# vrenkens/tfkaldi

Measured on AMD Instinct MI355X. Metric: acoustic frames/sec (train step), higher is better.
Workload: dtype f32 emulated (3xbf16 planes, 6 products, f32 accumulate)

## Files before the change

### tfkaldi_amd/csrc/gemm_bf16.hip

```cpp
#include "gemm_bf16.h"
#include "x3_layout.h"

#include <math.h>
#include <stdlib.h>
#include <string.h>

#include <type_traits>

namespace tfk {
namespace {

typedef __bf16 bf16x8 __attribute__((ext_vector_type(8)));
typedef __bf16 bf16x4 __attribute__((ext_vector_type(4)));
typedef float f32x16 __attribute__((ext_vector_type(16)));
typedef uint32_t u32x4 __attribute__((ext_vector_type(4)));
typedef int i32x4 __attribute__((ext_vector_type(4)));

constexpr int BK = 64;
constexpr int kOOB = (int)0x80000000;
constexpr int NUM_XCD = 8;

__device__ __forceinline__ void tile_of_block(int tiles_m, int tiles_n, int group_rows, int bid, int& tm, int& tn) {
  const int nwg = tiles_m * tiles_n;
  const int xcd = bid % NUM_XCD, loc = bid / NUM_XCD;
  const int q = nwg / NUM_XCD, r = nwg % NUM_XCD;
  const int seq = (xcd < r ? xcd * (q + 1) : r * (q + 1) + (xcd - r) * q) + loc;
  const int per_group = group_rows * tiles_n;
  const int grp = seq / per_group;
  const int first_m = grp * group_rows;
  const int gsize = min(group_rows, tiles_m - first_m);
  const int within = seq - grp * per_group;
  tm = first_m + within % gsize;
  tn = within / gsize;
}

__device__ __forceinline__ uint16_t f2bf(float x) { return __builtin_bit_cast(uint16_t, (__bf16)x); }

template <int EPI, int WAVES_M, int WAVES_N, int FM, int FN>
__device__ __forceinline__ void epilogue(const GemmArgsB& p, f32x16 (&acc)[FM][FN], int tiles_m, int tm, int m0, int n0,
                                         int wm, int wn, int i, int h, float* red) {
  constexpr int BM = WAVES_M * FM * 32, BN = WAVES_N * FN * 32;
  auto row_of = [&](int a, int r) { return m0 + (wm * FM + a) * 32 + 4 * h + (r & 3) + 8 * (r >> 2); };
#pragma unroll
  for (int b = 0; b < FN; ++b) {
    const int cidx = (wn * FN + b) * 32 + i;
    const int col = n0 + cidx;
    const bool col_ok = col < p.N;
    const int colc = col_ok ? col : p.N - 1;
    if constexpr ((EPI & EPI_BIAS) != 0) {
      const float bv = p.bias[colc];
#pragma unroll
      for (int a = 0; a < FM; ++a)
#pragma unroll
        for (int r = 0; r < 16; ++r) acc[a][b][r] += bv;
    }
    if constexpr ((EPI & EPI_EVAL_ACT) != 0) {
      const bool bn = p.act_mean != nullptr;
      const float mu = bn ? p.act_mean[colc] : 0.f;
      const float rs = bn ? rsqrtf(p.act_rstd[colc] + p.bn_eps) : 1.f;
      const float be = bn ? p.act_beta[colc] : 0.f;
#pragma unroll
      for (int a = 0; a < FM; ++a)
#pragma unroll
        for (int r = 0; r < 16; ++r) {
          float u = acc[a][b][r];
          if (bn) u = (u - mu) * rs + be;
          switch (p.act_nonlin) {
            case 0: u = fmaxf(u, 0.f); break;
            case 1: u = 1.f / (1.f + expf(-u)); break;
            case 2: u = tanhf(u); break;
            default: break;
          }
          acc[a][b][r] = u;
        }
    }
    if constexpr ((EPI & EPI_COLSTATS) != 0) {
      const int vlim = p.row_vend ? min(p.M, p.row_vend[m0 >> 6]) : p.M;
      const int n_tile = max(1, min(BM, vlim - m0));
      float cmean = 0.f;
#pragma unroll
      for (int pass = 0; pass < 2; ++pass) {
        float s = 0.f;
#pragma unroll
        for (int a = 0; a < FM; ++a)
#pragma unroll
          for (int r = 0; r < 16; ++r) {
            const float v = acc[a][b][r];
            if (row_of(a, r) < vlim) s += pass == 0 ? v : (v - cmean) * (v - cmean);
          }
        s += __shfl_xor(s, 32);
        if (h == 0) red[wm * BN + cidx] = s;
        __syncthreads();
        float t = 0.f;
#pragma unroll
        for (int w = 0; w < WAVES_M; ++w) t += red[w * BN + cidx];
        if (pass == 0) {
          cmean = t / (float)n_tile;
        } else if (wm == 0 && h == 0 && col_ok) {
          p.stats[((size_t)0 * tiles_m + tm) * p.ldc + col] = cmean;
          p.stats[((size_t)1 * tiles_m + tm) * p.ldc + col] = t;
        }
        __syncthreads();
      }
    }
    if constexpr ((EPI & EPI_DACT) != 0) {
      const float mu = p.act_mean[colc], rsd = p.act_rstd[colc];
      const float dscale = p.act_scale > 0.f ? p.act_scale : 1.f;
      const bool from_a = p.act_nonlin == 0 && p.act_beta != nullptr;
      const float be = from_a ? p.act_beta[colc] : 0.f;
      const float keep = p.act_keep > 0.f ? p.act_keep : 1.f;
      float s1 = 0.f, s2 = 0.f;
#pragma unroll
      for (int a = 0; a < FM; ++a) {
        float av[16], zv[16];
#pragma unroll
        for (int r = 0; r < 16; ++r) {
          const int row = min(row_of(a, r), p.M - 1);
          av[r] = p.act_a[(size_t)row * p.ldc + colc];
        }
        if (!from_a) {
#pragma unroll
          for (int r = 0; r < 16; ++r) {
            const int row = min(row_of(a, r), p.M - 1);
            zv[r] = p.act_z[(size_t)row * p.ldc + colc];
          }
        }
#pragma unroll
        for (int r = 0; r < 16; ++r) {
          float d1;
          switch (p.act_nonlin) {
            case 0: d1 = av[r] > 0.f ? dscale : 0.f; break;
            case 1: d1 = av[r] * (1.f - av[r]); break;
            case 2: d1 = 1.f - av[r] * av[r]; break;
            default: d1 = 1.f;
          }
          const float du = acc[a][b][r] * d1;
          acc[a][b][r] = du;
          if (row_of(a, r) < p.M) {
            s1 += du;
            s2 += du * (from_a ? av[r] * keep - be : (zv[r] - mu) * rsd);
          }
        }
      }
      s1 += __shfl_xor(s1, 32);
      s2 += __shfl_xor(s2, 32);
      if (h == 0) {
        red[(0 * WAVES_M + wm) * BN + cidx] = s1;
        red[(1 * WAVES_M + wm) * BN + cidx] = s2;
      }
      __syncthreads();
      if (wm == 0 && h == 0 && col_ok) {
        float t1 = 0.f, t2 = 0.f;
#pragma unroll
        for (int w = 0; w < WAVES_M; ++w) {
          t1 += red[(0 * WAVES_M + w) * BN + cidx];
          t2 += red[(1 * WAVES_M + w) * BN + cidx];
        }
        p.stats[((size_t)0 * p.stats_stride + tm) * p.ldc + col] = t1;
        p.stats[((size_t)1 * p.stats_stride + tm) * p.ldc + col] = t2;
      }
      __syncthreads();
    }
#pragma unroll
    for (int a = 0; a < FM; ++a) {
      float old[16];
      if constexpr ((EPI & EPI_ACCUM) != 0) {
#pragma unroll
        for (int r = 0; r < 16; ++r) old[r] = p.C[(size_t)min(row_of(a, r), p.M - 1) * p.ldc + colc];
      }
#pragma unroll
      for (int r = 0; r < 16; ++r) {
        const int row = row_of(a, r);
        float v = acc[a][b][r];
        if (EPI & EPI_ACCUM) v += old[r];
        if (col_ok && row < p.M) {
          p.C[(size_t)row * p.ldc + col] = v;
          if constexpr ((EPI & EPI_EVAL_ACT) != 0) {
            if (p.C_twin) {
              if (p.ct_x3) {
                const size_t at = x3::at((size_t)row, col, p.ldct);
                uint16_t q0, q1, q2;
                x3::split3(v, q0, q1, q2);
                p.C_twin[at] = (bf16_t)q0;
                p.C_twin[at + 64] = (bf16_t)q1;
                p.C_twin[at + 128] = (bf16_t)q2;
              } else {
                p.C_twin[(size_t)row * p.ldct + col] = f2bf(v);
              }
            }
          }
        }
      }
    }
  }
}


template <int EXT>
__device__ __forceinline__ int ks_swz(int r) {
  return EXT == 64 ? (((r >> 1) & 1) << 2) : ((r & 3) << 2);
}

template <bool KC, int EXT, int NTH, int BKT = 64>
struct DmaOperand {
  static_assert(BKT == 64 || BKT == 32, "ring slot of 64 or 32 k");
  static constexpr int NP = EXT * BKT / 8 / NTH;
  static_assert((EXT * BKT / 8) % NTH == 0 && NP >= 1, "pieces per thread");
  i32x4 rsrc;
  int voff[NP];
  int kidx[NP];
  int kstride;
  int k_lim;

  __device__ __forceinline__ void init(const bf16_t* base, int ld, int rows, int ext0, int ext_lim, int k_lim_,
                                       int tid, long extra_bytes = 0) {
    const unsigned long long a = (unsigned long long)base;
    rsrc[0] = (int)(unsigned)a;
    rsrc[1] = (int)((unsigned)(a >> 32) & 0xffffu);
    rsrc[2] = (int)(rows * ld * 2 + extra_bytes);
    rsrc[3] = 0x00020000;
    k_lim = k_lim_;
    kstride = KC ? 2 : ld * 2;
#pragma unroll
    for (int j = 0; j < NP; ++j) {
      const int idx = tid + j * NTH;
      if (KC) {
        constexpr int CPR = BKT / 8;
        const int r = idx / CPR;
        const int sw = BKT == 64 ? ((r >> 1) & 7) : ((r >> 2) & 3);
        const int k = ((idx % CPR) ^ sw) << 3;
        const int e = ext0 + r;
        voff[j] = e < ext_lim ? (e * ld + k) * 2 : kOOB;
        kidx[j] = k;
      } else {
        constexpr int CH = EXT / 8;
        const int r = idx / CH;
        const int c = (idx % CH) ^ ks_swz<EXT>(r);
        const int e = ext0 + (c << 3);
        voff[j] = e < ext_lim ? (r * ld + e) * 2 : kOOB;
        kidx[j] = r;
      }
    }
  }
  __device__ __forceinline__ void issue(int j, unsigned image, int k0, int wave, int plane_bytes = 0) const {
    const int off = (k0 + kidx[j] < k_lim) ? voff[j] : kOOB;
    const unsigned dst = image + (unsigned)(wave * 64 + j * NTH) * 16u;
    const int soff = k0 * kstride + plane_bytes;
    asm volatile("s_mov_b32 m0, %0\n\ts_nop 0\n\tbuffer_load_dwordx4 %1, %2, %3 offen lds"
                 :
                 : "s"(dst), "v"(off), "s"(rsrc), "s"(soff)
                 : "memory");
  }
};

template <bool KC, int EXT, int NF, int BKT = 64>
struct Frag {
  int off[KC ? 4 : NF];
  __device__ __forceinline__ void init(int lane, int frag0) {
    if constexpr (KC) {
      const int i = lane & 31, kb = lane >> 5, sw = BKT == 64 ? ((i >> 1) & 7) : ((i >> 2) & 3);
#pragma unroll
      for (int ks = 0; ks < BKT / 16; ++ks) off[ks] = (frag0 * 32 + i) * (BKT * 2) + ((((2 * ks + kb) ^ sw)) << 4);
    } else {
      constexpr int ROWB = EXT * 2;
      const int kb = lane >> 5, half = (lane >> 4) & 1, j = (lane >> 2) & 3, q = lane & 3;
      const int jj = EXT == 64 ? (j >> 1) : j;
#pragma unroll
      for (int f = 0; f < NF; ++f)
        off[f] = (8 * kb + j) * ROWB + ((4 * ((frag0 + f) ^ jj) + 2 * half + (q >> 1)) << 4) + ((q & 1) << 3);
    }
  }
  __device__ __forceinline__ bf16x8 read(const char* img, int f, int ks) const {
    if constexpr (KC) {
      return *reinterpret_cast<const bf16x8*>(img + off[ks] + f * 32 * (BKT * 2));
    } else {
      constexpr int ROWB = EXT * 2;
      typedef __attribute__((address_space(3))) bf16x4 lds_bf16x4;
      const char* q = img + off[f] + ks * 16 * ROWB;
      const bf16x4 lo = __builtin_amdgcn_ds_read_tr16_b64_v4bf16((lds_bf16x4*)q);
      const bf16x4 hi = __builtin_amdgcn_ds_read_tr16_b64_v4bf16((lds_bf16x4*)(q + 4 * ROWB));
      return __builtin_shufflevector(lo, hi, 0, 1, 2, 3, 4, 5, 6, 7);
    }
  }
};

template <bool KC, int EXT, int NTH>
struct DmaOperand3 {
  static constexpr int NP = EXT * 12 / NTH;
  static_assert((EXT * 12) % NTH == 0 && NP >= 1, "pieces per thread");
  i32x4 rsrc;
  int voff[NP];
  int kidx[NP];
  int kstride;
  int k_lim;

  __device__ __forceinline__ void init(const bf16_t* base, int ld, int rows, int ext0, int ext_lim, int k_lim_, int tid) {
    const unsigned long long a = (unsigned long long)base;
    rsrc[0] = (int)(unsigned)a;
    rsrc[1] = (int)((unsigned)(a >> 32) & 0xffffu);
    rsrc[2] = (int)(x3::elems((size_t)rows, ld) * 2);
    rsrc[3] = 0x00020000;
    k_lim = k_lim_;
    kstride = KC ? 12 : ld * 6;
#pragma unroll
    for (int j = 0; j < NP; ++j) {
      const int n = tid + j * NTH;
      if (KC) {
        int r, q, c;
        x3::kc_decode(n, r, q, c);
        const int e = ext0 + r;
        voff[j] = e < ext_lim ? (int)(x3::at((size_t)e, c * 8, ld) + q * 64) * 2 : kOOB;
        kidx[j] = c * 8;
      } else {
        int r, b, q, e8;
        x3::ks_decode<EXT>(n, r, b, q, e8);
        const int e = ext0 + b * 32 + e8 * 8;
        voff[j] = e < ext_lim ? (int)(x3::at((size_t)r, e, ld) + q * 64) * 2 : kOOB;
        kidx[j] = r;
      }
    }
  }
  template <bool GUARD>
  __device__ __forceinline__ void issue(int j, unsigned image, int k0, int wave) const {
    const int off = (!GUARD || k0 + kidx[j] < k_lim) ? voff[j] : kOOB;
    const unsigned dst = image + (unsigned)(wave * 64 + j * NTH) * 16u;
    const int soff = k0 * kstride;
    asm volatile("s_mov_b32 m0, %0\n\ts_nop 0\n\tbuffer_load_dwordx4 %1, %2, %3 offen lds"
                 :
                 : "s"(dst), "v"(off), "s"(rsrc), "s"(soff)
                 : "memory");
  }
};

template <bool KC, int EXT, int NF>
struct Frag3 {
  int off[2];
  __device__ __forceinline__ void init(int lane, int frag0) {
#pragma unroll
    for (int v = 0; v < 2; ++v) off[v] = KC ? x3::kc_lane_off(lane, frag0, v) : x3::ks_lane_off<EXT>(lane, frag0, v);
  }
  __device__ __forceinline__ Frag3 at(int bytes) const {
    Frag3 r;
    r.off[0] = off[0] + bytes;
    r.off[1] = off[1] + bytes;
    return r;
  }
  __device__ __forceinline__ bf16x8 read(const char* img, int f, int ks, int pl) const {
    if constexpr (KC) {
      return *reinterpret_cast<const bf16x8*>(img + off[ks] + x3::kc_imm(f, pl));
    } else {
      typedef __attribute__((address_space(3))) bf16x4 lds_bf16x4;
      const int X = 3 * f + pl;
      const char* q = img + off[X & 1];
      const bf16x4 lo = __builtin_amdgcn_ds_read_tr16_b64_v4bf16((lds_bf16x4*)(q + x3::ks_imm<EXT>(X, ks, 0)));
      const bf16x4 hi = __builtin_amdgcn_ds_read_tr16_b64_v4bf16((lds_bf16x4*)(q + x3::ks_imm<EXT>(X, ks, 1)));
      return __builtin_shufflevector(lo, hi, 0, 1, 2, 3, 4, 5, 6, 7);
    }
  }
};

template <bool KC, int EXT, int NF16>
struct Frag3M {
  int off[KC ? 1 : 4];
  __device__ __forceinline__ void init(int lane, int frag0) {
    if constexpr (KC) {
      off[0] = x3::kc16_lane_off(lane, frag0);
    } else {
#pragma unroll
      for (int v = 0; v < 4; ++v) off[v] = x3::ks16_lane_off<EXT>(lane, frag0, v & 1, v >> 1);
    }
  }
  __device__ __forceinline__ Frag3M at(int bytes) const {
    Frag3M r;
#pragma unroll
    for (int v = 0; v < (KC ? 1 : 4); ++v) r.off[v] = off[v] + bytes;
    return r;
  }
  __device__ __forceinline__ bf16x8 read(const char* img, int f, int pl) const {
    if constexpr (KC) {
      return *reinterpret_cast<const bf16x8*>(img + off[0] + x3::kc16_imm(f, pl));
    } else {
      typedef __attribute__((address_space(3))) bf16x4 lds_bf16x4;
      const int X = 3 * (f >> 1) + pl;
      const char* q = img + off[(X & 1) + 2 * (f & 1)];
      const bf16x4 lo = __builtin_amdgcn_ds_read_tr16_b64_v4bf16((lds_bf16x4*)(q + x3::ks16_imm<EXT>(X, 0)));
      const bf16x4 hi = __builtin_amdgcn_ds_read_tr16_b64_v4bf16((lds_bf16x4*)(q + x3::ks16_imm<EXT>(X, 1)));
      return __builtin_shufflevector(lo, hi, 0, 1, 2, 3, 4, 5, 6, 7);
    }
  }
};

#ifndef TFKB_ABL
#define TFKB_ABL 0
#endif

#define TFKB_WAIT_BARRIER(n) \
  asm volatile("s_waitcnt vmcnt(%0)\n\ts_waitcnt lgkmcnt(0)\n\ts_barrier" : : "n"(n) : "memory")

constexpr int kSplitFlagWords = 4096;
constexpr int kSplitXccWord = 2048;
template <bool A_KC, bool B_KC, int EPI, int WAVES_M, int WAVES_N, int FM, int FN, int NS, int BKT = 64, int SCHED = 0,
          int NPL = 1, int KSPLIT = 1, int LOADERS = 0>
__device__ __forceinline__ void dma_tile(const GemmArgsB& p, int tiles_m, int tiles_n, int group_rows, int bid, char* smem) {
  static_assert(LOADERS == 0 || (NPL == 3 && LOADERS == WAVES_M * WAVES_N), "loader waves: one per multiplying wave, x3 only");
  constexpr int NTH = WAVES_M * WAVES_N * 64;
  constexpr int BM = WAVES_M * FM * 32, BN = WAVES_N * FN * 32;
  typedef typename std::conditional<NPL == 3, DmaOperand3<A_KC, BM, NTH>, DmaOperand<A_KC, BM, NTH, BKT>>::type OA;
  typedef typename std::conditional<NPL == 3, DmaOperand3<B_KC, BN, NTH>, DmaOperand<B_KC, BN, NTH, BKT>>::type OB;
  constexpr int A_BYTES = BM * BKT * 2, B_BYTES = BN * BKT * 2, STAGE = NPL * (A_BYTES + B_BYTES);
  constexpr int NPA = OA::NP, NPB = OB::NP, NP = OA::NP + OB::NP;
  constexpr int KSPT = BKT / 16;
  static_assert(KSPT == 4 || KSPT == 2, "ring slot of 64 or 32 k");
  static_assert(NS >= 3 && (NS - 2) * NP + (NPL == 3 ? NP / 2 : 0) <= 63, "ring depth / vmcnt range");
  static_assert(FM * FN >= 2 || NPL == 3, "two independent accumulator chains per wave");
  static_assert(NPL == 1 || (NPL == 3 && SCHED == 0), "planes");
  static_assert(KSPLIT == 1 || (KSPLIT == 2 && NPL == 3), "split-K: the fp32-emulating contraction only");

  const int tid = threadIdx.x;
  const int lane = tid & 63;
  const int i = lane & 31, h = lane >> 5;
  const int wave = __builtin_amdgcn_readfirstlane(tid >> 6);
  const int wm = wave / WAVES_N, wn = wave % WAVES_N;
  int tm, tn;
  const int khalf = KSPLIT == 2 ? (bid / NUM_XCD) & 1 : 0;
  const int tile_bid = KSPLIT == 2 ? (bid / NUM_XCD >> 1) * NUM_XCD + bid % NUM_XCD : bid;
  tile_of_block(tiles_m, tiles_n, group_rows, tile_bid, tm, tn);
  const int m0 = tm * BM, n0 = tn * BN;
  unsigned my_xcc = 0;
  if constexpr (KSPLIT == 2) {
    if (p.splitk_local) {
      asm volatile("s_getreg_b32 %0, hwreg(HW_REG_XCC_ID, 0, 4)" : "=s"(my_xcc));
      if (tid == 0)
        __hip_atomic_store(reinterpret_cast<unsigned*>(p.splitk_ws) + kSplitXccWord + 2 * (tm * tiles_n + tn) + khalf, my_xcc + 1,
                           __ATOMIC_RELAXED, __HIP_MEMORY_SCOPE_AGENT);
    }
  }

  const int K8 = (p.K + 7) & ~7;
  const int nk_all = (p.K + BKT - 1) / BKT;
  const int h0 = KSPLIT == 2 ? max(1, (nk_all + 1) / 2 - p.splitk_skew) : nk_all;
  const int kbase = khalf ? h0 : 0;
  const int nk = KSPLIT == 2 ? (khalf ? nk_all - h0 : h0) : nk_all;
  const int k_end = (kbase + nk) * BKT;
  const unsigned lds0 = __builtin_amdgcn_readfirstlane((unsigned)(unsigned long long)smem);
  OA la;
  OB lb;
  const int a_klim = min(A_KC ? K8 : p.K, k_end), b_klim = min(B_KC ? K8 : p.K, k_end);
  const int nk_full = min(a_klim, b_klim) / BKT - kbase;
  if constexpr (LOADERS > 0) {
    if (wave >= WAVES_M * WAVES_N) {
      const int lwave = wave - WAVES_M * WAVES_N;
      la.init(p.A, p.lda, A_KC ? p.M : p.K, m0, A_KC ? p.M : ((p.M + 7) & ~7), a_klim, tid - NTH);
      lb.init(p.B, p.ldb, B_KC ? p.N : p.K, n0, B_KC ? p.N : ((p.N + 7) & ~7), b_klim, tid - NTH);
      auto tile = [&](auto guard, int slot, int kt) {
        if (TFKB_ABL & 2) return;
#pragma unroll
        for (int j = 0; j < NPA; ++j)
          la.template issue<decltype(guard)::value>(j, lds0 + (unsigned)(slot * STAGE), (kt + kbase) * BKT, lwave);
#pragma unroll
        for (int j = 0; j < NPB; ++j)
          lb.template issue<decltype(guard)::value>(j, lds0 + (unsigned)(slot * STAGE + NPL * A_BYTES), (kt + kbase) * BKT, lwave);
      };
#pragma unroll
      for (int t = 0; t < NS - 1; ++t) tile(std::true_type(), t, t);
      TFKB_WAIT_BARRIER((NS - 2) * NP);
      int ws = NS - 1;
      const int n_fast = max(0, min(nk, nk_full - (NS - 1)));
#pragma unroll 1
      for (int kt = 0; kt < nk; ++kt) {
        if (kt < n_fast) tile(std::false_type(), ws, kt + NS - 1);
        else tile(std::true_type(), ws, kt + NS - 1);
        TFKB_WAIT_BARRIER((NS - 2) * NP);
        ws = ws + 1 == NS ? 0 : ws + 1;
      }
      TFKB_WAIT_BARRIER(0);
      return;
    }
  } else {
    la.init(p.A, p.lda, A_KC ? p.M : p.K, m0, A_KC ? p.M : ((p.M + 7) & ~7), a_klim, tid);
    lb.init(p.B, p.ldb, B_KC ? p.N : p.K, n0, B_KC ? p.N : ((p.N + 7) & ~7), b_klim, tid);
  }
  typename std::conditional<NPL == 3, Frag3<A_KC, BM, FM>, Frag<A_KC, BM, FM, BKT>>::type qa;
  typename std::conditional<NPL == 3, Frag3<B_KC, BN, FN>, Frag<B_KC, BN, FN, BKT>>::type qb;
  qa.init(lane, wm * FM);
  qb.init(lane, wn * FN);

  f32x16 acc[FM][FN];
  f32x16 acc2[NPL == 3 ? FM : 1][NPL == 3 ? FN : 1];
#pragma unroll
  for (int a = 0; a < FM; ++a)
#pragma unroll
    for (int b = 0; b < FN; ++b)
#pragma unroll
      for (int r = 0; r < 16; ++r) acc[a][b][r] = 0.f;
  if constexpr (NPL == 3) {
#pragma unroll
    for (int a = 0; a < FM; ++a)
#pragma unroll
      for (int b = 0; b < FN; ++b)
#pragma unroll
        for (int r = 0; r < 16; ++r) acc2[a][b][r] = 0.f;
  }

  auto piece_g = [&](auto guard, int j, int slot, int kt) {
    if (TFKB_ABL & 2) return;
    if constexpr (LOADERS > 0) {
      return;
    } else if constexpr (NPL == 3) {
      if (j < NPA)
        la.template issue<decltype(guard)::value>(j, lds0 + (unsigned)(slot * STAGE), (kt + kbase) * BKT, wave);
      else
        lb.template issue<decltype(guard)::value>(j - NPA, lds0 + (unsigned)(slot * STAGE + NPL * A_BYTES), (kt + kbase) * BKT, wave);
    } else {
      if (j < NPA)
        la.issue(j, lds0 + (unsigned)(slot * STAGE), (kt + kbase) * BKT, wave);
      else
        lb.issue(j - NPA, lds0 + (unsigned)(slot * STAGE + A_BYTES), (kt + kbase) * BKT, wave);
    }
  };
  auto piece = [&](int j, int slot, int kt) { piece_g(std::true_type(), j, slot, kt); };
#pragma unroll
  for (int t = 0; t < NS - 1; ++t)
#pragma unroll
    for (int j = 0; j < NP; ++j) piece(j, t, t);
  constexpr int NPH = NPL == 3 ? NP / 2 : 0;
#pragma unroll
  for (int j = 0; j < NPH; ++j) piece(j, NS - 1, NS - 1);
  TFKB_WAIT_BARRIER((NS - 2) * NP + NPH);

  bf16x8 fa[2][NPL][FM], fb[2][NPL][FN];
  auto read_frags = [&](int buf, const char* st, int ks) {
    if (TFKB_ABL & 4) return;
#pragma unroll
    for (int pl = 0; pl < NPL; ++pl) {
      if constexpr (NPL == 3) {
#pragma unroll
        for (int a = 0; a < FM; ++a) fa[buf][pl][a] = qa.read(st, a, ks, pl);
#pragma unroll
        for (int b = 0; b < FN; ++b) fb[buf][pl][b] = qb.read(st + NPL * A_BYTES, b, ks, pl);
      } else {
#pragma unroll
        for (int a = 0; a < FM; ++a) fa[buf][pl][a] = qa.read(st, a, ks);
#pragma unroll
        for (int b = 0; b < FN; ++b) fb[buf][pl][b] = qb.read(st + A_BYTES, b, ks);
      }
    }
  };
  if (TFKB_ABL & 4) {
#pragma unroll
    for (int q = 0; q < 2; ++q) {
#pragma unroll
      for (int pl = 0; pl < NPL; ++pl) {
#pragma unroll
        for (int a = 0; a < FM; ++a)
#pragma unroll
          for (int e = 0; e < 8; ++e) fa[q][pl][a][e] = (__bf16)(float)(lane + e + pl);
#pragma unroll
        for (int b = 0; b < FN; ++b)
#pragma unroll
          for (int e = 0; e < 8; ++e) fb[q][pl][b][e] = (__bf16)(float)(lane - e - pl);
      }
    }
  }
  auto mfma_step = [&](int cur) {
    if (TFKB_ABL & 1) {
#pragma unroll
      for (int pl = 0; pl < NPL; ++pl) {
#pragma unroll
        for (int a = 0; a < FM; ++a) asm volatile("" : : "v"(fa[cur][pl][a]));
#pragma unroll
        for (int b = 0; b < FN; ++b) asm volatile("" : : "v"(fb[cur][pl][b]));
      }
    } else if constexpr (NPL == 1) {
#pragma unroll
      for (int a = 0; a < FM; ++a)
#pragma unroll
        for (int b = 0; b < FN; ++b)
          acc[a][b] = __builtin_amdgcn_mfma_f32_32x32x16_bf16(fa[cur][0][a], fb[cur][0][b], acc[a][b], 0, 0, 0);
    } else {
      constexpr int PA[6] = {2, 1, 0, 1, 0, 0}, PB[6] = {0, 1, 2, 0, 1, 0};
#pragma unroll
      for (int c = 0; c < 5; ++c)
#pragma unroll
        for (int a = 0; a < FM; ++a)
#pragma unroll
          for (int b = 0; b < FN; ++b)
            acc2[a][b] = __builtin_amdgcn_mfma_f32_32x32x16_bf16(fa[cur][PA[c]][a], fb[cur][PB[c]][b], acc2[a][b], 0, 0, 0);
#pragma unroll
      for (int a = 0; a < FM; ++a)
#pragma unroll
        for (int b = 0; b < FN; ++b)
          acc[a][b] = __builtin_amdgcn_mfma_f32_32x32x16_bf16(fa[cur][0][a], fb[cur][0][b], acc[a][b], 0, 0, 0);
    }
  };
  int rs = 0, ws = NS - 1;
  if constexpr (SCHED == 2) {
    static_assert(WAVES_M * WAVES_N == 8, "two waves per SIMD");
    const int group = wave >> 2;
    bf16x8 wa[KSPT][FM], wb[KSPT][FN];
    if (group == 1) {
      __builtin_amdgcn_sched_barrier(0);
      asm volatile("s_barrier" : : : "memory");
      __builtin_amdgcn_sched_barrier(0);
    }
#pragma unroll 1
    for (int kt = 0; kt < nk; ++kt) {
      const char* st = smem + rs * STAGE;
#pragma unroll
      for (int ks = 0; ks < KSPT; ++ks) {
#pragma unroll
        for (int a = 0; a < FM; ++a) wa[ks][a] = qa.read(st, a, ks);
#pragma unroll
        for (int b = 0; b < FN; ++b) wb[ks][b] = qb.read(st + A_BYTES, b, ks);
      }
#pragma unroll
      for (int j = 0; j < NP; ++j) piece(j, ws, kt + NS - 1);
      __builtin_amdgcn_sched_barrier(0);
      TFKB_WAIT_BARRIER((NS - 2) * NP);
      __builtin_amdgcn_sched_barrier(0);
#pragma unroll
      for (int ks = 0; ks < KSPT; ++ks)
#pragma unroll
        for (int a = 0; a < FM; ++a)
#pragma unroll
          for (int b = 0; b < FN; ++b)
            acc[a][b] = __builtin_amdgcn_mfma_f32_32x32x16_bf16(wa[ks][a], wb[ks][b], acc[a][b], 0, 0, 0);
      rs = rs + 1 == NS ? 0 : rs + 1;
      ws = ws + 1 == NS ? 0 : ws + 1;
      __builtin_amdgcn_sched_barrier(0);
      asm volatile("s_barrier" : : : "memory");
      __builtin_amdgcn_sched_barrier(0);
    }
    if (group == 0) {
      __builtin_amdgcn_sched_barrier(0);
      asm volatile("s_barrier" : : : "memory");
      __builtin_amdgcn_sched_barrier(0);
    }
  } else if constexpr (NPL == 3 && TFK_X3_M16 != 0) {
    static_assert(KSPT == 2, "fp32-emulating contraction: 32 k per ring slot");
    constexpr int FM16 = 2 * FM, FN16 = 2 * FN;
    typedef float f32x4 __attribute__((ext_vector_type(4)));
    Frag3M<A_KC, BM, FM16> ma;
    Frag3M<B_KC, BN, FN16> mb;
    ma.init(lane, wm * FM16);
    mb.init(lane, wn * FN16);
    f32x4 c1[FM16][FN16], c2[FM16][FN16];
#pragma unroll
    for (int a = 0; a < FM16; ++a)
#pragma unroll
      for (int b = 0; b < FN16; ++b) {
        c1[a][b] = f32x4{0.f, 0.f, 0.f, 0.f};
        c2[a][b] = f32x4{0.f, 0.f, 0.f, 0.f};
      }
    bf16x8 ga[3][FM16], gb[3][FN16], gb0n[FN16];
    auto rd_a = [&](const decltype(ma)& r, int pl) {
#pragma unroll
      for (int a = 0; a < FM16; ++a) ga[pl][a] = r.read(smem, a, pl);
    };
    auto rd_b = [&](const decltype(mb)& r, int pl, bf16x8 (&dst)[FN16]) {
#pragma unroll
      for (int b = 0; b < FN16; ++b) dst[b] = r.read(smem, b, pl);
    };
    auto mm = [&](int pa, int pb) {
#pragma unroll
      for (int a = 0; a < FM16; ++a)
#pragma unroll
        for (int b = 0; b < FN16; ++b) {
          if (pa + pb == 0) c1[a][b] = __builtin_amdgcn_mfma_f32_16x16x32_bf16(ga[0][a], gb[0][b], c1[a][b], 0, 0, 0);
          else c2[a][b] = __builtin_amdgcn_mfma_f32_16x16x32_bf16(ga[pa][a], gb[pb][b], c2[a][b], 0, 0, 0);
        }
      __builtin_amdgcn_sched_barrier(0);
    };
    auto pieces = [&](auto guard, int part, int j0, int j1, int slot, int tile) {
#pragma unroll
      for (int j = j0 + part * (j1 - j0) / 3; j < j0 + (part + 1) * (j1 - j0) / 3; ++j) piece_g(guard, j, slot, tile);
    };
    {
      const auto r0a = ma.at(0);
      const auto r0b = mb.at(NPL * A_BYTES);
      rd_a(r0a, 0);
      rd_b(r0b, 0, gb[0]);
      rd_b(r0b, 1, gb[1]);
      rd_b(r0b, 2, gb[2]);
    }
    const int n_fast = max(0, min(nk, nk_full - NS));
    auto iteration = [&](auto guard, int kt) {
      const auto ra = ma.at(rs * STAGE);
      rd_a(ra, 1);
      pieces(guard, 0, NPH, NP, ws, kt + NS - 1);
      mm(0, 0);
      rd_a(ra, 2);
      pieces(guard, 1, NPH, NP, ws, kt + NS - 1);
      mm(0, 1);
      pieces(guard, 2, NPH, NP, ws, kt + NS - 1);
      mm(0, 2);
      TFKB_WAIT_BARRIER((NS - 2) * NP);
      rs = rs + 1 == NS ? 0 : rs + 1;
      ws = ws + 1 == NS ? 0 : ws + 1;
      const bool fetch = kt + 1 < nk;
      const auto na = ma.at(rs * STAGE);
      const auto nb = mb.at(rs * STAGE + NPL * A_BYTES);
      if (fetch) {
        rd_a(na, 0);
        rd_b(nb, 0, gb0n);
      }
      pieces(guard, 0, 0, NPH, ws, kt + NS);
      mm(1, 0);
      if (fetch) rd_b(nb, 2, gb[2]);
      pieces(guard, 1, 0, NPH, ws, kt + NS);
      mm(1, 1);
      if (fetch) rd_b(nb, 1, gb[1]);
      pieces(guard, 2, 0, NPH, ws, kt + NS);
      mm(2, 0);
      if (fetch) {
#pragma unroll
        for (int b = 0; b < FN16; ++b) gb[0][b] = gb0n[b];
      }
    };
#pragma unroll 1
    for (int kt = 0; kt < n_fast; ++kt) iteration(std::false_type(), kt);
#pragma unroll 1
    for (int kt = n_fast; kt < nk; ++kt) iteration(std::true_type(), kt);
    {
      const int src = (16 * h + (i & 15)) * 4;
#pragma unroll
      for (int a = 0; a < FM; ++a)
#pragma unroll
        for (int b = 0; b < FN; ++b)
#pragma unroll
          for (int r = 0; r < 16; ++r) {
            const int addr = src + (((r >> 2) & 1) ? 128 : 0);
            const f32x4& t0 = c1[2 * a + (r >> 3)][2 * b], &u0 = c2[2 * a + (r >> 3)][2 * b];
            const f32x4& t1 = c1[2 * a + (r >> 3)][2 * b + 1], &u1 = c2[2 * a + (r >> 3)][2 * b + 1];
            const float v0 = __builtin_bit_cast(float, __builtin_amdgcn_ds_bpermute(addr, __builtin_bit_cast(int, t0[r & 3] + u0[r & 3])));
            const float v1 = __builtin_bit_cast(float, __builtin_amdgcn_ds_bpermute(addr, __builtin_bit_cast(int, t1[r & 3] + u1[r & 3])));
            acc[a][b][r] = (i & 16) ? v1 : v0;
          }
    }
  } else if constexpr (NPL == 3) {
    static_assert(KSPT == 2, "fp32-emulating contraction: 32 k per ring slot");
    constexpr int PA[6] = {2, 1, 0, 1, 0, 0}, PB[6] = {0, 1, 2, 0, 1, 0};
    auto step3 = [&](auto guard, int cur, bool fetch, const decltype(qa)& ra, const decltype(qb)& rb, int nks, int j0, int j1,
                     int slot, int tile) {
#pragma unroll
      for (int c = 0; c < 6; ++c) {
        if (c < 3 && fetch && !(TFKB_ABL & 4)) {
#pragma unroll
          for (int a = 0; a < FM; ++a) fa[cur ^ 1][PA[c]][a] = ra.read(smem, a, nks, PA[c]);
#pragma unroll
          for (int b = 0; b < FN; ++b) fb[cur ^ 1][PB[c]][b] = rb.read(smem, b, nks, PB[c]);
        }
#pragma unroll
        for (int j = j0 + c * (j1 - j0) / 6; j < j0 + (c + 1) * (j1 - j0) / 6; ++j) piece_g(guard, j, slot, tile);
        if (TFKB_ABL & 1) {
#pragma unroll
          for (int a = 0; a < FM; ++a) asm volatile("" : : "v"(fa[cur][PA[c]][a]));
#pragma unroll
          for (int b = 0; b < FN; ++b) asm volatile("" : : "v"(fb[cur][PB[c]][b]));
        } else {
#pragma unroll
          for (int a = 0; a < FM; ++a)
#pragma unroll
            for (int b = 0; b < FN; ++b) {
              if (c < 5)
                acc2[a][b] = __builtin_amdgcn_mfma_f32_32x32x16_bf16(fa[cur][PA[c]][a], fb[cur][PB[c]][b], acc2[a][b], 0, 0, 0);
              else
                acc[a][b] = __builtin_amdgcn_mfma_f32_32x32x16_bf16(fa[cur][PA[c]][a], fb[cur][PB[c]][b], acc[a][b], 0, 0, 0);
            }
        }
        __builtin_amdgcn_sched_barrier(0);
      }
    };
    read_frags(0, smem, 0);
    const int n_fast = max(0, min(nk, nk_full - NS));
    auto iteration = [&](auto guard, int kt) {
      const auto ra = qa.at(rs * STAGE);
      const auto rb = qb.at(rs * STAGE + NPL * A_BYTES);
      step3(guard, 0, true, ra, rb, 1, NPH, NP, ws, kt + NS - 1);
      TFKB_WAIT_BARRIER((NS - 2) * NP);
      rs = rs + 1 == NS ? 0 : rs + 1;
      ws = ws + 1 == NS ? 0 : ws + 1;
      const auto na = qa.at(rs * STAGE);
      const auto nb = qb.at(rs * STAGE + NPL * A_BYTES);
      step3(guard, 1, kt + 1 < nk, na, nb, 0, 0, NPH, ws, kt + NS);
    };
#pragma unroll 1
    for (int kt = 0; kt < n_fast; ++kt) iteration(std::false_type(), kt);
#pragma unroll 1
    for (int kt = n_fast; kt < nk; ++kt) iteration(std::true_type(), kt);
  } else {
  read_frags(0, smem, 0);
#pragma unroll 1
  for (int kt = 0; kt < nk; ++kt) {
    const char* st = smem + rs * STAGE;
#pragma unroll
    for (int ks = 0; ks < KSPT - 1; ++ks) {
      const int cur = ks & 1;
      read_frags(cur ^ 1, st, ks + 1);
#pragma unroll
      for (int j = ks * NP / (KSPT - 1); j < (ks + 1) * NP / (KSPT - 1); ++j) piece(j, ws, kt + NS - 1);
      mfma_step(cur);
      __builtin_amdgcn_sched_barrier(0);
    }
    TFKB_WAIT_BARRIER((NS - 2) * NP);
    rs = rs + 1 == NS ? 0 : rs + 1;
    ws = ws + 1 == NS ? 0 : ws + 1;
    if (kt + 1 < nk) read_frags(0, smem + rs * STAGE, 0);
    mfma_step((KSPT - 1) & 1);
    __builtin_amdgcn_sched_barrier(0);
  }
  }
  TFKB_WAIT_BARRIER(0);
  if constexpr (NPL == 3) {
#pragma unroll
    for (int a = 0; a < FM; ++a)
#pragma unroll
      for (int b = 0; b < FN; ++b)
#pragma unroll
        for (int r = 0; r < 16; ++r) acc[a][b][r] += acc2[a][b][r];
  }
  if constexpr (KSPLIT == 2) {
    typedef float f32x4 __attribute__((ext_vector_type(4)));
    unsigned* flags = reinterpret_cast<unsigned*>(p.splitk_ws);
    const int tile = tm * tiles_n + tn;
    constexpr int kSys = 1 | (1 << 4);
    __amdgpu_buffer_rsrc_t part = __builtin_amdgcn_make_buffer_rsrc(
        (void*)(p.splitk_ws + kSplitFlagWords + (size_t)tile * (BM * BN)), 0, BM * BN * 4, 0x00020000);
    unsigned* sh = reinterpret_cast<unsigned*>(smem);
    if (tid == 0) {
      sh[0] = __hip_atomic_fetch_add(&flags[2 * tile], 1u, __ATOMIC_RELAXED, __HIP_MEMORY_SCOPE_AGENT);
      sh[1] = p.splitk_local ? __hip_atomic_load(&flags[kSplitXccWord + 2 * tile + (khalf ^ 1)], __ATOMIC_RELAXED, __HIP_MEMORY_SCOPE_AGENT)
                             : 0u;
    }
    __syncthreads();
    const bool first = sh[0] == 0;
    if (first) {
      const bool same_xcd = p.splitk_local && sh[1] == my_xcc + 1;
      if (same_xcd) {
#pragma unroll
        for (int a = 0; a < FM; ++a)
#pragma unroll
          for (int b = 0; b < FN; ++b)
#pragma unroll
            for (int q = 0; q < 4; ++q)
              __builtin_amdgcn_raw_buffer_store_b128(
                  __builtin_bit_cast(u32x4, f32x4{acc[a][b][4 * q], acc[a][b][4 * q + 1], acc[a][b][4 * q + 2], acc[a][b][4 * q + 3]}),
                  part, ((((wave * FM + a) * FN + b) * 4 + q) * 64 + lane) * 16, 0, 0);
      } else {
#pragma unroll
        for (int a = 0; a < FM; ++a)
#pragma unroll
          for (int b = 0; b < FN; ++b)
#pragma unroll
            for (int q = 0; q < 4; ++q)
              __builtin_amdgcn_raw_buffer_store_b128(
                  __builtin_bit_cast(u32x4, f32x4{acc[a][b][4 * q], acc[a][b][4 * q + 1], acc[a][b][4 * q + 2], acc[a][b][4 * q + 3]}),
                  part, ((((wave * FM + a) * FN + b) * 4 + q) * 64 + lane) * 16, 0, kSys);
      }
      asm volatile("s_waitcnt vmcnt(0)" : : : "memory");
      __syncthreads();
      if (tid == 0) __hip_atomic_store(&flags[2 * tile + 1], 1u, __ATOMIC_RELAXED, __HIP_MEMORY_SCOPE_AGENT);
      return;
    }
    if (tid == 0) {
      int spin = 0;
      for (; spin < (1 << 23) && __hip_atomic_load(&flags[2 * tile + 1], __ATOMIC_RELAXED, __HIP_MEMORY_SCOPE_AGENT) == 0; ++spin)
        __builtin_amdgcn_s_sleep(2);
      if (spin == (1 << 23) && p.err) __hip_atomic_store(p.err, 1u, __ATOMIC_RELAXED, __HIP_MEMORY_SCOPE_SYSTEM);
      __hip_atomic_store(&flags[2 * tile], 0u, __ATOMIC_RELAXED, __HIP_MEMORY_SCOPE_AGENT);
      __hip_atomic_store(&flags[2 * tile + 1], 0u, __ATOMIC_RELAXED, __HIP_MEMORY_SCOPE_AGENT);
      __hip_atomic_store(&flags[kSplitXccWord + 2 * tile], 0u, __ATOMIC_RELAXED, __HIP_MEMORY_SCOPE_AGENT);
      __hip_atomic_store(&flags[kSplitXccWord + 2 * tile + 1], 0u, __ATOMIC_RELAXED, __HIP_MEMORY_SCOPE_AGENT);
    }
    __syncthreads();
#pragma unroll
    for (int a = 0; a < FM; ++a)
#pragma unroll
      for (int b = 0; b < FN; ++b)
#pragma unroll
        for (int q = 0; q < 4; ++q) {
          const f32x4 o = __builtin_bit_cast(
              f32x4, __builtin_amdgcn_raw_buffer_load_b128(part, ((((wave * FM + a) * FN + b) * 4 + q) * 64 + lane) * 16, 0, kSys));
          acc[a][b][4 * q] += o.x;
          acc[a][b][4 * q + 1] += o.y;
          acc[a][b][4 * q + 2] += o.z;
          acc[a][b][4 * q + 3] += o.w;
        }
    __syncthreads();
  }
  epilogue<EPI, WAVES_M, WAVES_N, FM, FN>(p, acc, tiles_m, tm, m0, n0, wm, wn, i, h, reinterpret_cast<float*>(smem));
}

template <bool A_KC, bool B_KC, int EPI, int WAVES_M, int WAVES_N, int FM, int FN, int NS, int BKT = 64, int SCHED = 0,
          int NPL = 1, int KSPLIT = 1, int LOADERS = 0>
__global__ void __launch_bounds__((WAVES_M * WAVES_N + LOADERS) * 64)
gemm_bf16_dma_kernel(GemmArgsB p, int tiles_m, int tiles_n, int group_rows) {
  extern __shared__ __attribute__((aligned(16))) char smem[];
  dma_tile<A_KC, B_KC, EPI, WAVES_M, WAVES_N, FM, FN, NS, BKT, SCHED, NPL, KSPLIT, LOADERS>(p, tiles_m, tiles_n, group_rows,
                                                                                            blockIdx.x, smem);
}

template <int EPI_NT, int EPI_TN, int GWM, int GWN, int GFM, int GFN, int GNS, int HWM, int HWN, int HFM, int HFN, int HNS,
          int HBK>
__global__ void __launch_bounds__(GWM * GWN * 64)
gemm_bf16_dual_kernel(GemmArgsB p1, GemmArgsB p2, int tiles_m1, int tiles_n1, int group1, int tiles_m2, int tiles_n2,
                      int group2) {
  static_assert(GWM * GWN == HWM * HWN, "both halves run on the same block size");
  extern __shared__ __attribute__((aligned(16))) char smem[];
  const int n1 = tiles_m1 * tiles_n1;
  if ((int)blockIdx.x < n1)
    dma_tile<true, true, EPI_NT, GWM, GWN, GFM, GFN, GNS>(p1, tiles_m1, tiles_n1, group1, blockIdx.x, smem);
  else
    dma_tile<false, false, EPI_TN, HWM, HWN, HFM, HFN, HNS, HBK, (HBK == 32 ? 2 : 0)>(p2, tiles_m2, tiles_n2, group2, blockIdx.x - n1,
                                                                                      smem);
}

constexpr int NT = 256, PF = 4;
constexpr int KC_LD = BK + 8;

template <bool KC, int EXT>
struct Operand {
  static constexpr int LD = KC ? KC_LD : EXT + 32;
  static constexpr int SZ = (KC ? EXT : BK) * LD;
  static constexpr int NCH = EXT * BK / 8 / NT;
};

template <bool KC, int EXT>
struct Loader {
  static constexpr int NCH = Operand<KC, EXT>::NCH;
  __amdgpu_buffer_rsrc_t rsrc;
  int voff[NCH];
  int kidx[NCH];
  int kstride;
  int k_lim;

  static __device__ __forceinline__ void coords(int c, int& r, int& q) {
    if (KC) { r = c >> 3; q = (c & 7) << 3; }
    else { r = c / (EXT / 8); q = (c % (EXT / 8)) << 3; }
  }
  __device__ __forceinline__ void init(const bf16_t* base, int ld, int rows, int ext0, int ext_lim, int k_lim_,
                                       int tid) {
    rsrc = __builtin_amdgcn_make_buffer_rsrc((void*)base, 0, rows * ld * 2, 0x00020000);
    k_lim = k_lim_;
    kstride = KC ? 2 : ld * 2;
#pragma unroll
    for (int j = 0; j < NCH; ++j) {
      int r, q;
      coords(tid + j * NT, r, q);
      if (KC) {
        voff[j] = (ext0 + r < ext_lim) ? ((ext0 + r) * ld + q) * 2 : kOOB;
        kidx[j] = q;
      } else {
        voff[j] = (ext0 + q < ext_lim) ? (r * ld + ext0 + q) * 2 : kOOB;
        kidx[j] = r;
      }
    }
  }
  __device__ __forceinline__ void load(u32x4 (&v)[NCH], int k0) const {
#pragma unroll
    for (int j = 0; j < NCH; ++j) {
      const int off = (k0 + kidx[j] < k_lim) ? voff[j] : kOOB;
      v[j] = __builtin_amdgcn_raw_buffer_load_b128(rsrc, off, k0 * kstride, 0);
    }
  }
  __device__ __forceinline__ void store(const u32x4 (&v)[NCH], bf16_t* s, int tid) const {
#pragma unroll
    for (int j = 0; j < NCH; ++j) {
      int r, q;
      coords(tid + j * NT, r, q);
      *reinterpret_cast<u32x4*>(s + r * Operand<KC, EXT>::LD + q) = v[j];
    }
  }
};

template <bool KC, int LD>
__device__ __forceinline__ bf16x8 fragment(const bf16_t* s, int ext_base, int ks, int lane) {
  if (KC) {
    const int i = lane & 31, kb = lane >> 5;
    return *reinterpret_cast<const bf16x8*>(s + (ext_base + i) * LD + 16 * ks + 8 * kb);
  } else {
    const int kb = lane >> 5, half = (lane >> 4) & 1, j = (lane >> 2) & 3, q = lane & 3;
    const bf16_t* p = s + (16 * ks + 8 * kb + j) * LD + ext_base + 16 * half + 4 * q;
    typedef __attribute__((address_space(3))) bf16x4 lds_bf16x4;
    const bf16x4 lo = __builtin_amdgcn_ds_read_tr16_b64_v4bf16((lds_bf16x4*)p);
    const bf16x4 hi = __builtin_amdgcn_ds_read_tr16_b64_v4bf16((lds_bf16x4*)(p + 4 * LD));
    return __builtin_shufflevector(lo, hi, 0, 1, 2, 3, 4, 5, 6, 7);
  }
}

template <bool A_KC, bool B_KC, int EPI, int FM, int FN>
__global__ void __launch_bounds__(NT)
gemm_bf16_kernel(GemmArgsB p, int tiles_m, int tiles_n, int group_rows) {
  extern __shared__ __attribute__((aligned(16))) bf16_t smem_e[];
  bf16_t* smem = smem_e;
  constexpr int BM = 64 * FM, BN = 64 * FN;
  typedef Operand<A_KC, BM> OA;
  typedef Operand<B_KC, BN> OB;
  constexpr int A_SZ = OA::SZ, B_SZ = OB::SZ, STAGE = A_SZ + B_SZ;
  constexpr int KSTEPS = BK / 16;

  const int tid = threadIdx.x;
  const int lane = tid & 63;
  const int i = lane & 31, h = lane >> 5;
  const int wave = __builtin_amdgcn_readfirstlane(tid >> 6);
  const int wm = wave >> 1, wn = wave & 1;
  int tm, tn;
  tile_of_block(tiles_m, tiles_n, group_rows, blockIdx.x, tm, tn);
  const int m0 = tm * BM, n0 = tn * BN;

  const int K8 = (p.K + 7) & ~7;
  Loader<A_KC, BM> la;
  Loader<B_KC, BN> lb;
  la.init(p.A, p.lda, A_KC ? p.M : p.K, m0, A_KC ? p.M : ((p.M + 7) & ~7), A_KC ? K8 : p.K, tid);
  lb.init(p.B, p.ldb, B_KC ? p.N : p.K, n0, B_KC ? p.N : ((p.N + 7) & ~7), B_KC ? K8 : p.K, tid);

  constexpr bool ALT = FM * FN == 1;
  f32x16 acc[FM][FN], acc_alt;
#pragma unroll
  for (int r = 0; r < 16; ++r) acc_alt[r] = 0.f;
#pragma unroll
  for (int a = 0; a < FM; ++a)
#pragma unroll
    for (int b = 0; b < FN; ++b)
#pragma unroll
      for (int r = 0; r < 16; ++r) acc[a][b][r] = 0.f;

  const int nk = (p.K + BK - 1) / BK;
  u32x4 ra[PF][OA::NCH], rb[PF][OB::NCH];
#pragma unroll
  for (int j = 0; j < PF; ++j) {
    la.load(ra[j], j * BK);
    lb.load(rb[j], j * BK);
  }
  bf16_t* st0 = smem;
  bf16_t* st1 = smem + STAGE;
  bf16_t* st2 = smem + 2 * STAGE;
  la.store(ra[0], st0, tid);
  lb.store(rb[0], st0 + A_SZ, tid);
  la.store(ra[1], st1, tid);
  lb.store(rb[1], st1 + A_SZ, tid);
  la.load(ra[0], PF * BK);
  lb.load(rb[0], PF * BK);
  la.load(ra[1], (PF + 1) * BK);
  lb.load(rb[1], (PF + 1) * BK);
  __syncthreads();
  bf16x8 fa[2][FM], fb[2][FN];
  auto read_frags = [&](int buf, const bf16_t* st, int ks) {
#pragma unroll
    for (int a = 0; a < FM; ++a) fa[buf][a] = fragment<A_KC, OA::LD>(st, wm * 32 * FM + a * 32, ks, lane);
#pragma unroll
    for (int b = 0; b < FN; ++b) fb[buf][b] = fragment<B_KC, OB::LD>(st + A_SZ, wn * 32 * FN + b * 32, ks, lane);
  };
  read_frags(0, st0, 0);
#pragma unroll 1
  for (int kt0 = 0; kt0 < nk; kt0 += PF) {
#pragma unroll
    for (int j = 0; j < PF; ++j) {
      const int kt = kt0 + j;
      const int s2 = (j + 2) % PF;
      la.store(ra[s2], st2, tid);
      lb.store(rb[s2], st2 + A_SZ, tid);
      la.load(ra[s2], (kt + 2 + PF) * BK);
      lb.load(rb[s2], (kt + 2 + PF) * BK);
#pragma unroll
      for (int ks = 0; ks < KSTEPS; ++ks) {
        const int cur = ks & 1;
        if (ks + 1 < KSTEPS) read_frags(cur ^ 1, st0, ks + 1);
        else read_frags(cur ^ 1, st1, 0);
        if (ALT && (ks & 1)) {
          acc_alt = __builtin_amdgcn_mfma_f32_32x32x16_bf16(fa[cur][0], fb[cur][0], acc_alt, 0, 0, 0);
        } else {
#pragma unroll
          for (int a = 0; a < FM; ++a)
#pragma unroll
            for (int b = 0; b < FN; ++b)
              acc[a][b] = __builtin_amdgcn_mfma_f32_32x32x16_bf16(fa[cur][a], fb[cur][b], acc[a][b], 0, 0, 0);
        }
      }
      __syncthreads();
      bf16_t* t = st0; st0 = st1; st1 = st2; st2 = t;
    }
  }
  if constexpr (ALT) {
#pragma unroll
    for (int r = 0; r < 16; ++r) acc[0][0][r] += acc_alt[r];
  }
  epilogue<EPI, 2, 2, FM, FN>(p, acc, tiles_m, tm, m0, n0, wm, wn, i, h, reinterpret_cast<float*>(smem));
}

template <int EPI_NT, int EPI_TN, int WN>
__global__ void __launch_bounds__(WN == 2 ? 256 : 512)
gemm_bf16x3_dual_kernel(GemmArgsB p1, GemmArgsB p2, int tiles_m1, int tiles_n1, int group1, int tiles_m2, int tiles_n2, int group2,
                        int tn_first) {
  extern __shared__ __attribute__((aligned(16))) char smem[];
  const int n1 = tiles_m1 * tiles_n1, n2 = tiles_m2 * tiles_n2;
  const int b = blockIdx.x;
  const bool nt = tn_first ? b >= n2 : b < n1;
  if (nt)
    dma_tile<true, true, EPI_NT, 2, WN ? WN : 2, 2, WN ? 4 / WN : 2, 3, 32, 0, 3, 1, WN ? 0 : 4>(p1, tiles_m1, tiles_n1, group1,
                                                                                              tn_first ? b - n2 : b, smem);
  else
    dma_tile<false, false, EPI_TN, 2, WN ? WN : 2, 2, WN ? 4 / WN : 2, 3, 32, 0, 3, 1, WN ? 0 : 4>(p2, tiles_m2, tiles_n2, group2,
                                                                                                tn_first ? b : b - n1, smem);
}

struct CfgB {
  int bm, bn;
};
const CfgB kCfgB[kNumGemmBf16Configs] = {{64, 64}, {128, 64}, {128, 128}, {128, 64}, {128, 128}, {256, 128}, {128, 64}, {256, 128},
                                         {256, 256}};
int g_forced_b = -2;
int g_group_rows = 0;

template <class Kern>
int launch_grid(Kern kern, const GemmArgsB& p, int bm, int bn, int threads, size_t lds, hipStream_t stream, bool* attr_done,
                int blocks_per_tile = 1) {
  const int tiles_m = (p.M + bm - 1) / bm, tiles_n = (p.N + bn - 1) / bn;
  if (!*attr_done) {
    hipError_t e = hipFuncSetAttribute(reinterpret_cast<const void*>(kern), hipFuncAttributeMaxDynamicSharedMemorySize,
                                       160 * 1024);
    if (e != hipSuccess) return (int)e;
    *attr_done = true;
  }
  int group_rows = g_group_rows;
  if (group_rows <= 0) {
    const double per_xcd = (double)tiles_m * tiles_n / NUM_XCD;
    group_rows = (int)(sqrt(per_xcd * bn / bm) + 0.5);
  }
  if (group_rows < 1) group_rows = 1;
  if (group_rows > tiles_m) group_rows = tiles_m;
  hipLaunchKernelGGL(kern, dim3(tiles_m * tiles_n * blocks_per_tile), dim3(threads), lds, stream, p, tiles_m, tiles_n, group_rows);
  return (int)hipGetLastError();
}

template <bool A_KC, bool B_KC, int EPI, int FM, int FN>
int launch_reg(const GemmArgsB& p, hipStream_t stream) {
  constexpr int BM = 64 * FM, BN = 64 * FN;
  const size_t lds = (size_t)3 * (Operand<A_KC, BM>::SZ + Operand<B_KC, BN>::SZ) * sizeof(bf16_t);
  static bool attr_done = false;
  return launch_grid(&gemm_bf16_kernel<A_KC, B_KC, EPI, FM, FN>, p, BM, BN, NT, lds, stream, &attr_done);
}
template <bool A_KC, bool B_KC, int EPI, int WAVES_M, int WAVES_N, int FM, int FN, int NS, int BKT = 64, int SCHED = 0,
          int NPL = 1, int KSPLIT = 1, int LOADERS = 0>
int launch_dma(const GemmArgsB& p, hipStream_t stream) {
  constexpr int BM = WAVES_M * FM * 32, BN = WAVES_N * FN * 32;
  const size_t lds = (size_t)NS * NPL * (BM + BN) * BKT * 2;
  static_assert((size_t)NS * NPL * (BM + BN) * BKT * 2 <= 160 * 1024, "LDS");
  static bool attr_done = false;
  return launch_grid(&gemm_bf16_dma_kernel<A_KC, B_KC, EPI, WAVES_M, WAVES_N, FM, FN, NS, BKT, SCHED, NPL, KSPLIT, LOADERS>, p,
                     BM, BN, (WAVES_M * WAVES_N + LOADERS) * 64, lds, stream, &attr_done, KSPLIT);
}

int g_x3_cfg = -2;
int x3_cfg() {
  if (g_x3_cfg == -2) {
    const char* q = getenv("TFK_BF16X3_CFG");
    g_x3_cfg = q ? atoi(q) : -1;
  }
  return g_x3_cfg;
}
bool x3_split_shape(bool tn, int M, int N, int K) {
  const long tiles = (long)((M + 127) / 128) * ((N + 127) / 128);
  return !tn && tiles >= 64 && tiles < 200 && tiles % NUM_XCD == 0 && 2 * tiles <= kSplitXccWord && K >= 512;
}
bool x3_split_shape_tn(int M, int N, int K) {
  const long m128 = (M + 127) / 128, tiles128 = m128 * ((N + 127) / 128), tiles64 = m128 * ((N + 63) / 64);
  return tiles128 < 100 && tiles64 >= 64 && tiles64 < 200 && tiles64 % NUM_XCD == 0 && 2 * tiles64 <= kSplitXccWord && K >= 512;
}
int x3_waves() {
  static const int w = [] {
    const char* q = getenv("TFK_BF16X3_WAVES");
    const int v = q ? atoi(q) : 8;
    return v == 4 || v == 44 ? v : 8;
  }();
  return w;
}
int x3_handover_local() {
  static const int v = [] {
    const char* q = getenv("TFK_X3_HANDOVER");
    return (q && !strcmp(q, "l2")) ? 1 : 0;
  }();
  return v;
}
int x3_kskew() {
  static const int v = [] {
    const char* q = getenv("TFK_X3_KSKEW");
    const int k = q ? atoi(q) : 1;
    return k < 0 ? 0 : k > 8 ? 8 : k;
  }();
  return v;
}
template <bool A_KC, bool B_KC, int EPI>
int launch_x3(const GemmArgsB& p_in, hipStream_t stream) {
  GemmArgsB p = p_in;
  p.splitk_local = x3_handover_local();
  p.splitk_skew = x3_kskew();
  const int forced = x3_cfg();
  const long m128 = (p.M + 127) / 128, n128 = (p.N + 127) / 128;
  const int wv = x3_waves();
  if constexpr (A_KC) {
    if ((forced == 2 || forced < 0) && p.splitk_ws && x3_split_shape(false, p.M, p.N, p.K) &&
        p.splitk_ws_floats >= (size_t)kSplitFlagWords + (size_t)m128 * n128 * 128 * 128)
      return wv == 8    ? launch_dma<A_KC, B_KC, EPI, 2, 4, 2, 1, 3, 32, 0, 3, 2>(p, stream)
             : wv == 44 ? launch_dma<A_KC, B_KC, EPI, 2, 2, 2, 2, 3, 32, 0, 3, 2, 4>(p, stream)
                        : launch_dma<A_KC, B_KC, EPI, 2, 2, 2, 2, 3, 32, 0, 3, 2>(p, stream);
  } else {
    if ((forced == 3 || (forced < 0 && p.K < 2048)) && m128 * n128 < 100 && (long)((p.M + 63) / 64) * ((p.N + 63) / 64) >= 192)
      return launch_dma<A_KC, B_KC, EPI, 2, 2, 1, 1, 4, 32, 0, 3>(p, stream);
    if ((forced == 2 || forced < 0) && p.splitk_ws && x3_split_shape_tn(p.M, p.N, p.K) &&
        p.splitk_ws_floats >= (size_t)kSplitFlagWords + (size_t)m128 * ((p.N + 63) / 64) * 128 * 64)
      return launch_dma<A_KC, B_KC, EPI, 2, 2, 2, 1, 4, 32, 0, 3, 2>(p, stream);
  }
  const bool big = forced >= 0 ? forced == 1 : m128 * n128 >= 200;
  if (big)
    return wv == 8    ? launch_dma<A_KC, B_KC, EPI, 2, 4, 2, 1, 3, 32, 0, 3>(p, stream)
           : wv == 44 ? launch_dma<A_KC, B_KC, EPI, 2, 2, 2, 2, 3, 32, 0, 3, 1, 4>(p, stream)
                      : launch_dma<A_KC, B_KC, EPI, 2, 2, 2, 2, 3, 32, 0, 3>(p, stream);
  return launch_dma<A_KC, B_KC, EPI, 2, 2, 2, 1, 4, 32, 0, 3>(p, stream);
}

template <bool A_KC, bool B_KC, int EPI>
int launch(const GemmArgsB& p, hipStream_t stream) {
  int cfg = gemm_bf16_pick_config(p.M, p.N);
  if constexpr (!A_KC && !B_KC) {
    if (cfg == 8 || (g_forced_b < 0 && (long)((p.M + 255) / 256) * ((p.N + 255) / 256) >= 200))
      return launch_dma<false, false, EPI, 4, 2, 2, 4, 4, 32, 2>(p, stream);
  }
  if (cfg == 8) cfg = 5;
  switch (cfg) {
    case 0: return launch_reg<A_KC, B_KC, EPI, 1, 1>(p, stream);
    case 1: return launch_reg<A_KC, B_KC, EPI, 2, 1>(p, stream);
    case 2: return launch_reg<A_KC, B_KC, EPI, 2, 2>(p, stream);
    case 3: return launch_dma<A_KC, B_KC, EPI, 2, 2, 2, 1, 5>(p, stream);
    case 4: return launch_dma<A_KC, B_KC, EPI, 2, 2, 2, 2, 4>(p, stream);
    case 5: return launch_dma<A_KC, B_KC, EPI, 4, 2, 2, 2, 3>(p, stream);
    case 6: return launch_dma<A_KC, B_KC, EPI, 2, 2, 2, 1, 3>(p, stream);
    case 7: return launch_dma<A_KC, B_KC, EPI, 2, 2, 4, 2, 3>(p, stream);
  }
  return (int)hipErrorInvalidValue;
}

int pick_group_rows(int tiles_m, int tiles_n, int bm, int bn) {
  int group_rows = g_group_rows;
  if (group_rows <= 0) {
    const double per_xcd = (double)tiles_m * tiles_n / NUM_XCD;
    group_rows = (int)(sqrt(per_xcd * bn / bm) + 0.5);
  }
  if (group_rows < 1) group_rows = 1;
  if (group_rows > tiles_m) group_rows = tiles_m;
  return group_rows;
}

template <int EPI_NT, int EPI_TN, int GWM, int GWN, int GFM, int GFN, int GNS, int HWM, int HWN, int HFM, int HFN, int HNS, int HBK>
int launch_dual(const GemmArgsB& a, const GemmArgsB& w, hipStream_t stream) {
  constexpr int BMA = GWM * GFM * 32, BNA = GWN * GFN * 32, BMW = HWM * HFM * 32, BNW = HWN * HFN * 32;
  constexpr size_t lds_a = (size_t)GNS * (BMA + BNA) * 128, lds_w = (size_t)HNS * (BMW + BNW) * HBK * 2;
  constexpr size_t lds = lds_a > lds_w ? lds_a : lds_w;
  static_assert(lds <= 160 * 1024, "LDS");
  auto kern = &gemm_bf16_dual_kernel<EPI_NT, EPI_TN, GWM, GWN, GFM, GFN, GNS, HWM, HWN, HFM, HFN, HNS, HBK>;
  static bool attr_done = false;
  if (!attr_done) {
    hipError_t e = hipFuncSetAttribute(reinterpret_cast<const void*>(kern), hipFuncAttributeMaxDynamicSharedMemorySize,
                                       160 * 1024);
    if (e != hipSuccess) return (int)e;
    attr_done = true;
  }
  const int tma = (a.M + BMA - 1) / BMA, tna = (a.N + BNA - 1) / BNA, tmw = (w.M + BMW - 1) / BMW, tnw = (w.N + BNW - 1) / BNW;
  hipLaunchKernelGGL(kern, dim3(tma * tna + tmw * tnw), dim3(GWM * GWN * 64), lds, stream, a, w, tma, tna,
                     pick_group_rows(tma, tna, BMA, BNA), tmw, tnw, pick_group_rows(tmw, tnw, BMW, BNW));
  return (int)hipGetLastError();
}

template <int GWM, int GWN, int GFM, int GFN, int GNS, int HWM, int HWN, int HFM, int HFN, int HNS, int HBK>
int launch_dual_epi(const GemmArgsB& a, const GemmArgsB& w, hipStream_t stream) {
  const int key = (a.epi == EPI_DACT ? 2 : 0) + (w.epi == EPI_ACCUM ? 1 : 0);
  switch (key) {
    case 0: return launch_dual<0, 0, GWM, GWN, GFM, GFN, GNS, HWM, HWN, HFM, HFN, HNS, HBK>(a, w, stream);
    case 1: return launch_dual<0, EPI_ACCUM, GWM, GWN, GFM, GFN, GNS, HWM, HWN, HFM, HFN, HNS, HBK>(a, w, stream);
    case 2: return launch_dual<EPI_DACT, 0, GWM, GWN, GFM, GFN, GNS, HWM, HWN, HFM, HFN, HNS, HBK>(a, w, stream);
    default: return launch_dual<EPI_DACT, EPI_ACCUM, GWM, GWN, GFM, GFN, GNS, HWM, HWN, HFM, HFN, HNS, HBK>(a, w, stream);
  }
}

int g_dual_cfg = -2;

}

int gemm_bf16_dual_config(int M_nt, int N_nt, int M_tn, int N_tn) {
  if (g_dual_cfg == -2) {
    const char* q = getenv("TFK_BF16_DUAL_CFG");
    g_dual_cfg = q ? atoi(q) : -1;
  }
  if (g_dual_cfg == 0) return 0;
  if (g_dual_cfg == 3 || g_dual_cfg == 4 || g_dual_cfg == 5 || g_dual_cfg == 8) return g_dual_cfg;
  auto tiles = [](int M, int N, int bm, int bn) { return (long)((M + bm - 1) / bm) * ((N + bn - 1) / bn); };
  if (tiles(M_nt, N_nt, 256, 128) >= 200 && tiles(M_tn, N_tn, 256, 256) >= 200) return 8;
  if (tiles(M_nt, N_nt, 256, 128) + tiles(M_tn, N_tn, 256, 128) >= 512) return 5;
  if (tiles(M_nt, N_nt, 128, 128) + tiles(M_tn, N_tn, 128, 128) >= 256) return 4;
  if (tiles(M_nt, N_nt, 128, 64) + tiles(M_tn, N_tn, 128, 64) >= 256) return 3;
  return 0;
}
int gemm_bf16_dual_tile_rows(int cfg) { return (cfg == 5 || cfg == 8) ? 256 : (cfg == 3 || cfg == 4) ? 128 : 0; }

int gemm_bf16_dual(const GemmArgsB& nt, const GemmArgsB& tn, hipStream_t stream) {
  if (nt.M <= 0 || nt.N <= 0 || nt.K <= 0 || tn.M <= 0 || tn.N <= 0 || tn.K <= 0) return (int)hipErrorInvalidValue;
  if ((nt.lda & 7) || (nt.ldb & 7) || (nt.ldc & 3) || (tn.lda & 7) || (tn.ldb & 7) || (tn.ldc & 3)) return (int)hipErrorInvalidValue;
  if ((long)nt.M * nt.lda * 2 >= (1L << 31) || (long)nt.N * nt.ldb * 2 >= (1L << 31) ||
      (long)tn.K * tn.lda * 2 >= (1L << 31) || (long)tn.K * tn.ldb * 2 >= (1L << 31)) return (int)hipErrorInvalidValue;
  if ((nt.epi != 0 && nt.epi != EPI_DACT) || (tn.epi != 0 && tn.epi != EPI_ACCUM)) return -1;
  switch (gemm_bf16_dual_config(nt.M, nt.N, tn.M, tn.N)) {
    case 3: return launch_dual_epi<2, 2, 2, 1, 5, 2, 2, 2, 1, 5, 64>(nt, tn, stream);
    case 4: return launch_dual_epi<2, 2, 2, 2, 4, 2, 2, 2, 2, 4, 64>(nt, tn, stream);
    case 5: return launch_dual_epi<4, 2, 2, 2, 3, 4, 2, 2, 2, 3, 64>(nt, tn, stream);
    case 8: return launch_dual_epi<4, 2, 2, 2, 3, 4, 2, 2, 4, 4, 32>(nt, tn, stream);
  }
  return -1;
}

void gemm_bf16_force_config(int cfg) { g_forced_b = (cfg >= 0 && cfg < kNumGemmBf16Configs) ? cfg : -1; }

int gemm_bf16_pick_config(int M, int N) {
  if (g_forced_b == -2) {
    const char* q = getenv("TFK_BF16_CFG");
    const int v = q ? atoi(q) : -1;
    g_forced_b = (v >= 0 && v < kNumGemmBf16Configs) ? v : -1;
    if ((q = getenv("TFK_BF16_GROUP_ROWS"))) g_group_rows = atoi(q);
  }
  if (g_forced_b >= 0) return g_forced_b;
  const long m256 = (M + 255) / 256, m128 = (M + 127) / 128, n128 = (N + 127) / 128, n64 = (N + 63) / 64;
  if (m256 * n128 >= 200) return 5;
  if (m128 * n128 >= 200) return 4;
  return m128 * n64 > 256 ? 6 : 3;
}

int gemm_bf16_tile_rows(int M, int N) { return kCfgB[gemm_bf16_pick_config(M, N)].bm; }

size_t gemm_bf16x3_splitk_floats(GemmLayout layout, int M, int N, int K) {
  const int forced = x3_cfg();
  if (!(forced == 2 || forced < 0)) return 0;
  if (layout == GEMM_TN)
    return x3_split_shape_tn(M, N, K) ? (size_t)kSplitFlagWords + (size_t)((M + 127) / 128) * ((N + 63) / 64) * 128 * 64 : 0;
  if (!x3_split_shape(false, M, N, K)) return 0;
  return (size_t)kSplitFlagWords + (size_t)((M + 127) / 128) * ((N + 127) / 128) * 128 * 128;
}

namespace {
template <int EPI_NT, int EPI_TN, int WN>
int launch_x3_dual(const GemmArgsB& a, const GemmArgsB& w, hipStream_t stream) {
  constexpr size_t lds = (size_t)3 * 3 * (128 + 128) * 32 * 2;
  auto kern = &gemm_bf16x3_dual_kernel<EPI_NT, EPI_TN, WN>;
  static bool attr_done = false;
  if (!attr_done) {
    hipError_t e = hipFuncSetAttribute(reinterpret_cast<const void*>(kern), hipFuncAttributeMaxDynamicSharedMemorySize, 160 * 1024);
    if (e != hipSuccess) return (int)e;
    attr_done = true;
  }
  const int tma = (a.M + 127) / 128, tna = (a.N + 127) / 128, tmw = (w.M + 127) / 128, tnw = (w.N + 127) / 128;
  hipLaunchKernelGGL(kern, dim3(tma * tna + tmw * tnw), dim3(WN == 2 ? 256 : 512), lds, stream, a, w, tma, tna, pick_group_rows(tma, tna, 128, 128),
                     tmw, tnw, pick_group_rows(tmw, tnw, 128, 128), w.K > a.K ? 1 : 0);
  return (int)hipGetLastError();
}
bool x3_operands_ok(const GemmArgsB& p, long a_rows, long b_rows) {
  if (p.M <= 0 || p.N <= 0 || p.K <= 0 || (p.lda & 31) || (p.ldb & 31) || (p.ldc & 3)) return false;
  return (long)x3::elems(a_rows, p.lda) * 2 < (1L << 31) && (long)x3::elems(b_rows, p.ldb) * 2 < (1L << 31);
}
}

int gemm_bf16x3_dual(const GemmArgsB& nt, const GemmArgsB& tn, hipStream_t stream) {
  if (!x3_operands_ok(nt, nt.M, nt.N) || !x3_operands_ok(tn, tn.K, tn.K)) return (int)hipErrorInvalidValue;
  if ((nt.epi != 0 && nt.epi != EPI_DACT) || (tn.epi != 0 && tn.epi != EPI_ACCUM)) return -1;
  static const bool on = !getenv("TFK_BF16X3_DUAL") || atoi(getenv("TFK_BF16X3_DUAL")) != 0;
  const long tiles = (long)((nt.M + 127) / 128) * ((nt.N + 127) / 128) + (long)((tn.M + 127) / 128) * ((tn.N + 127) / 128);
  if (!on || tiles < 256) return -1;
  const int key = (nt.epi == EPI_DACT ? 2 : 0) + (tn.epi == EPI_ACCUM ? 1 : 0);
  switch (key) {
#define TFK_X3_DUAL(E1, E2)                                                                \
  (x3_waves() == 8    ? launch_x3_dual<E1, E2, 4>(nt, tn, stream)                            \
   : x3_waves() == 44 ? launch_x3_dual<E1, E2, 0>(nt, tn, stream)                            \
                      : launch_x3_dual<E1, E2, 2>(nt, tn, stream))
    case 0: return TFK_X3_DUAL(0, 0);
    case 1: return TFK_X3_DUAL(0, EPI_ACCUM);
    case 2: return TFK_X3_DUAL(EPI_DACT, 0);
    default: return TFK_X3_DUAL(EPI_DACT, EPI_ACCUM);
#undef TFK_X3_DUAL
  }
}

int gemm_bf16x3(GemmLayout layout, const GemmArgsB& p, hipStream_t stream) {
  if (p.M <= 0 || p.N <= 0 || p.K <= 0) return (int)hipErrorInvalidValue;
  if (!x3_operands_ok(p, layout == GEMM_TN ? p.K : p.M, layout == GEMM_NT ? p.N : p.K)) return (int)hipErrorInvalidValue;
  switch (layout) {
    case GEMM_NN:
      switch (p.epi) {
        case 0: return launch_x3<true, false, 0>(p, stream);
        case EPI_BIAS: return launch_x3<true, false, EPI_BIAS>(p, stream);
        case EPI_BIAS | EPI_COLSTATS: return launch_x3<true, false, EPI_BIAS | EPI_COLSTATS>(p, stream);
        case EPI_BIAS | EPI_EVAL_ACT: return launch_x3<true, false, EPI_BIAS | EPI_EVAL_ACT>(p, stream);
      }
      break;
    case GEMM_NT:
      if (p.epi == 0) return launch_x3<true, true, 0>(p, stream);
      if (p.epi == EPI_DACT) return launch_x3<true, true, EPI_DACT>(p, stream);
      break;
    case GEMM_TN:
      if (p.epi == 0) return launch_x3<false, false, 0>(p, stream);
      if (p.epi == EPI_ACCUM) return launch_x3<false, false, EPI_ACCUM>(p, stream);
      break;
  }
  return (int)hipErrorInvalidValue;
}

int gemm_bf16(GemmLayout layout, const GemmArgsB& p, hipStream_t stream) {
  if (p.M <= 0 || p.N <= 0 || p.K <= 0) return (int)hipErrorInvalidValue;
  if ((p.lda & 7) || (p.ldb & 7) || (p.ldc & 3)) return (int)hipErrorInvalidValue;
  {
    const long a_rows = layout == GEMM_TN ? p.K : p.M;
    const long b_rows = layout == GEMM_NT ? p.N : p.K;
    if (a_rows * p.lda * 2 >= (1L << 31) || b_rows * p.ldb * 2 >= (1L << 31)) return (int)hipErrorInvalidValue;
  }
  switch (layout) {
    case GEMM_NN:
      switch (p.epi) {
        case 0: return launch<true, false, 0>(p, stream);
        case EPI_BIAS: return launch<true, false, EPI_BIAS>(p, stream);
        case EPI_BIAS | EPI_COLSTATS: return launch<true, false, EPI_BIAS | EPI_COLSTATS>(p, stream);
        case EPI_BIAS | EPI_EVAL_ACT: return launch<true, false, EPI_BIAS | EPI_EVAL_ACT>(p, stream);
      }
      break;
    case GEMM_NT:
      if (p.epi == 0) return launch<true, true, 0>(p, stream);
      if (p.epi == EPI_DACT) return launch<true, true, EPI_DACT>(p, stream);
      break;
    case GEMM_TN:
      if (p.epi == 0) return launch<false, false, 0>(p, stream);
      if (p.epi == EPI_ACCUM) return launch<false, false, EPI_ACCUM>(p, stream);
      break;
  }
  return (int)hipErrorInvalidValue;
}

}
```

### tfkaldi_amd/csrc/x3_layout.h

```cpp
#pragma once
#include <stddef.h>
#include <stdint.h>

#if defined(__HIPCC__)
#define X3_HD __host__ __device__ __forceinline__
#else
#define X3_HD inline
#endif

namespace tfk {
namespace x3 {

constexpr int kSlotK = 32;

#ifndef TFK_X3_M16
#define TFK_X3_M16 0
#endif

X3_HD size_t elems(size_t rows, int ld) { return ((rows + 1) >> 1) * (size_t)(ld >> 5) * 192; }
X3_HD size_t at(size_t row, int col, int ld) {
  return ((row >> 1) * (size_t)(ld >> 5) + (size_t)(col >> 5)) * 192 + (row & 1) * 32 + (col & 31);
}

#if TFK_X3_M16
X3_HD int kc_swz(int r) { return ((r >> 3) & 1) * 3; }
#else
X3_HD int kc_swz(int r) { return (r >> 2) & 3; }
#endif
X3_HD void kc_decode(int n, int& r, int& q, int& c) {
  const int P = n / 24, rem = n - P * 24;
  q = rem >> 3;
  r = 2 * P + ((rem >> 2) & 1);
  c = (rem & 3) ^ kc_swz(r);
}
X3_HD int kc_addr(int r, int q, int c) { return (r >> 1) * 384 + q * 128 + (r & 1) * 64 + ((c ^ kc_swz(r)) << 4); }

template <int EXT>
X3_HD void ks_decode(int n, int& r, int& b, int& q, int& e8) {
  constexpr int CPP = EXT / 32 * 24;
  const int P = n / CPP, pos = n - P * CPP;
  const int nq = (pos >> 2) ^ ((P & 1) << 1);
  b = nq / 6;
  const int rem = nq - 6 * b;
  q = rem >> 1;
  r = 2 * P + (rem & 1);
#if TFK_X3_M16
  e8 = (pos & 3) ^ (((P >> 2) & 1) << 1);
#else
  e8 = pos & 3;
#endif
}
template <int EXT>
X3_HD int ks_addr(int r, int b, int q, int e8) {
  const int P = r >> 1;
#if TFK_X3_M16
  e8 ^= ((P >> 2) & 1) << 1;
#endif
  return P * (EXT / 32 * 384) + ((((6 * b + 2 * q + (r & 1)) ^ ((P & 1) << 1)) << 2) + e8) * 16;
}

X3_HD int kc_lane_off(int lane, int frag0, int ks) { return kc_addr(frag0 * 32 + (lane & 31), 0, 2 * ks + (lane >> 5)); }
X3_HD int kc_imm(int f, int q) { return f * (16 * 384) + q * 128; }
template <int EXT>
X3_HD int ks_lane_off(int lane, int frag0, int x_odd) {
  const int kb = lane >> 5, half = (lane >> 4) & 1, j = (lane >> 2) & 3, qq = lane & 3;
  const int t = (j >> 1) & 1;
  const int base = (4 * kb + (j >> 1)) * (EXT / 32 * 384) + (j & 1) * 64 + (2 * half + (qq >> 1)) * 16 + ((qq & 1) << 3) +
                   128 * 3 * frag0;
  const int xt_odd = (frag0 + x_odd) & 1;
  return base + (xt_odd ? -128 * t : 128 * t) + (x_odd ? 128 : 0);
}
template <int EXT>
X3_HD int ks_imm(int X, int ks, int hi) {
  return 128 * (X & ~1) + (ks * 8 + hi * 2) * (EXT / 32 * 384);
}

X3_HD int kc16_lane_off(int lane, int frag0) { return kc_addr(frag0 * 16 + (lane & 15), 0, lane >> 4); }
X3_HD int kc16_imm(int f, int q) { return f * (8 * 384) + q * 128; }
template <int EXT>
X3_HD int ks16_lane_off(int lane, int frag0, int x_odd, int f_odd) {
  const int g = lane >> 4, j = (lane >> 2) & 3, qq = lane & 3;
  const int t = (j >> 1) & 1;
  const int unit0 = frag0 >> 1;
  const int base = (4 * g + (j >> 1)) * (EXT / 32 * 384) + (j & 1) * 64 + ((f_odd ^ (g & 1)) << 5) + (qq >> 1) * 16 + ((qq & 1) << 3) +
                   128 * 3 * unit0;
  const int xt_odd = (unit0 + x_odd) & 1;
  return base + (xt_odd ? -128 * t : 128 * t) + (x_odd ? 128 : 0);
}
template <int EXT>
X3_HD int ks16_imm(int X, int hi) {
  return 128 * (X & ~1) + hi * 2 * (EXT / 32 * 384);
}

#if defined(__HIPCC__)
__device__ __forceinline__ void split3(float x, uint16_t& p1, uint16_t& p2, uint16_t& p3) {
  const uint32_t ux = __builtin_bit_cast(uint32_t, x);
  uint32_t b1 = (uint32_t)__builtin_bit_cast(uint16_t, (__bf16)x) << 16;
  const bool edge = (b1 & 0x7fffffffu) == 0x7f800000u && (ux & 0x7fffffffu) < 0x7f800000u;
  if (edge) b1 = ux & 0xffff0000u;
  const float r1 = x - __builtin_bit_cast(float, b1);
  uint32_t b2 = (uint32_t)__builtin_bit_cast(uint16_t, (__bf16)r1) << 16;
  if (edge) b2 = __builtin_bit_cast(uint32_t, r1) & 0xffff0000u;
  const float r2 = r1 - __builtin_bit_cast(float, b2);
  p1 = (uint16_t)(b1 >> 16);
  p2 = (uint16_t)(b2 >> 16);
  p3 = (uint16_t)(__builtin_bit_cast(uint32_t, r2) >> 16);
}
#endif

}
}
```

Measured before the change: 919,700.

## Pack short-K GEMM tiles into persistent tile lists in dual bf16x3 kernel

In the dual NT/TN fp32-emulating GEMM launch, the long-K GEMM keeps one tile per block while the short-K GEMM's tiles are grouped so that each block processes several consecutive tiles. The next tile's prologue is chained into the tail of the current one's k-loop. This is meant to balance per-block work between the two GEMMs and cut block count and pipeline fill/drain overhead. The epilogue also gets a buffer-resource store path with hardware bounds checking. The change adds complexity around reduction scratch LDS, tile switching mid-pipeline, and 2GB offset limits, which are now guarded.

```diff
diff --git a/tfkaldi_amd/csrc/gemm_bf16.hip b/tfkaldi_amd/csrc/gemm_bf16.hip
--- a/tfkaldi_amd/csrc/gemm_bf16.hip
+++ b/tfkaldi_amd/csrc/gemm_bf16.hip
@@ -20,11 +20,7 @@
 constexpr int kOOB = (int)0x80000000;
 constexpr int NUM_XCD = 8;
 
-__device__ __forceinline__ void tile_of_block(int tiles_m, int tiles_n, int group_rows, int bid, int& tm, int& tn) {
-  const int nwg = tiles_m * tiles_n;
-  const int xcd = bid % NUM_XCD, loc = bid / NUM_XCD;
-  const int q = nwg / NUM_XCD, r = nwg % NUM_XCD;
-  const int seq = (xcd < r ? xcd * (q + 1) : r * (q + 1) + (xcd - r) * q) + loc;
+__device__ __forceinline__ void tile_of_seq(int tiles_m, int tiles_n, int group_rows, int seq, int& tm, int& tn) {
   const int per_group = group_rows * tiles_n;
   const int grp = seq / per_group;
   const int first_m = grp * group_rows;
@@ -33,10 +29,17 @@
   tm = first_m + within % gsize;
   tn = within / gsize;
 }
+__device__ __forceinline__ void tile_of_block(int tiles_m, int tiles_n, int group_rows, int bid, int& tm, int& tn) {
+  const int nwg = tiles_m * tiles_n;
+  const int xcd = bid % NUM_XCD, loc = bid / NUM_XCD;
+  const int q = nwg / NUM_XCD, r = nwg % NUM_XCD;
+  const int seq = (xcd < r ? xcd * (q + 1) : r * (q + 1) + (xcd - r) * q) + loc;
+  tile_of_seq(tiles_m, tiles_n, group_rows, seq, tm, tn);
+}
 
 __device__ __forceinline__ uint16_t f2bf(float x) { return __builtin_bit_cast(uint16_t, (__bf16)x); }
 
-template <int EPI, int WAVES_M, int WAVES_N, int FM, int FN>
+template <int EPI, int WAVES_M, int WAVES_N, int FM, int FN, bool CBUF = false>
 __device__ __forceinline__ void epilogue(const GemmArgsB& p, f32x16 (&acc)[FM][FN], int tiles_m, int tm, int m0, int n0,
                                          int wm, int wn, int i, int h, float* red) {
   constexpr int BM = WAVES_M * FM * 32, BN = WAVES_N * FN * 32;
@@ -160,6 +163,30 @@
         p.stats[((size_t)1 * p.stats_stride + tm) * p.ldc + col] = t2;
       }
       __syncthreads();
+    }
+    if constexpr (CBUF) {
+      static_assert((EPI & EPI_EVAL_ACT) == 0, "no bf16 twin on this path");
+      const __amdgpu_buffer_rsrc_t crs =
+          __builtin_amdgcn_make_buffer_rsrc((void*)p.C, 0, (int)(((unsigned)(p.M - 1) * p.ldc + p.N) * 4u), 0x00020000);
+#pragma unroll
+      for (int a = 0; a < FM; ++a) {
+        const unsigned base = col_ok ? ((unsigned)(m0 + (wm * FM + a) * 32 + 4 * h) * p.ldc + col) * 4u : (unsigned)kOOB;
+        float old[16];
+        if constexpr ((EPI & EPI_ACCUM) != 0) {
+#pragma unroll
+          for (int r = 0; r < 16; ++r)
+            old[r] = __builtin_bit_cast(float, __builtin_amdgcn_raw_buffer_load_b32(
+                                                   crs, base + (unsigned)(((r & 3) + 8 * (r >> 2)) * p.ldc) * 4u, 0, 0));
+        }
+#pragma unroll
+        for (int r = 0; r < 16; ++r) {
+          float v = acc[a][b][r];
+          if (EPI & EPI_ACCUM) v += old[r];
+          __builtin_amdgcn_raw_buffer_store_b32(__builtin_bit_cast(unsigned, v), crs,
+                                                base + (unsigned)(((r & 3) + 8 * (r >> 2)) * p.ldc) * 4u, 0, 0);
+        }
+      }
+      continue;
     }
 #pragma unroll
     for (int a = 0; a < FM; ++a) {
@@ -394,15 +421,21 @@
 #define TFKB_ABL 0
 #endif
 
+#ifndef TFKB_TL
+#define TFKB_TL(ev, ti)
+#endif
+
 #define TFKB_WAIT_BARRIER(n) \
   asm volatile("s_waitcnt vmcnt(%0)\n\ts_waitcnt lgkmcnt(0)\n\ts_barrier" : : "n"(n) : "memory")
 
 constexpr int kSplitFlagWords = 4096;
 constexpr int kSplitXccWord = 2048;
 template <bool A_KC, bool B_KC, int EPI, int WAVES_M, int WAVES_N, int FM, int FN, int NS, int BKT = 64, int SCHED = 0,
-          int NPL = 1, int KSPLIT = 1, int LOADERS = 0>
-__device__ __forceinline__ void dma_tile(const GemmArgsB& p, int tiles_m, int tiles_n, int group_rows, int bid, char* smem) {
+          int NPL = 1, int KSPLIT = 1, int LOADERS = 0, bool LIST = false, bool CBUF = false>
+__device__ __forceinline__ void dma_tile(const GemmArgsB& p, int tiles_m, int tiles_n, int group_rows, int bid, char* smem,
+                                         int seq0 = 0, int ntiles = 1) {
   static_assert(LOADERS == 0 || (NPL == 3 && LOADERS == WAVES_M * WAVES_N), "loader waves: one per multiplying wave, x3 only");
+  static_assert(!LIST || (NPL == 3 && KSPLIT == 1 && LOADERS == 0), "tile lists: the unsplit fp32-emulating contraction, no loader waves");
   constexpr int NTH = WAVES_M * WAVES_N * 64;
   constexpr int BM = WAVES_M * FM * 32, BN = WAVES_N * FN * 32;
   typedef typename std::conditional<NPL == 3, DmaOperand3<A_KC, BM, NTH>, DmaOperand<A_KC, BM, NTH, BKT>>::type OA;
@@ -424,8 +457,9 @@
   int tm, tn;
   const int khalf = KSPLIT == 2 ? (bid / NUM_XCD) & 1 : 0;
   const int tile_bid = KSPLIT == 2 ? (bid / NUM_XCD >> 1) * NUM_XCD + bid % NUM_XCD : bid;
-  tile_of_block(tiles_m, tiles_n, group_rows, tile_bid, tm, tn);
-  const int m0 = tm * BM, n0 = tn * BN;
+  if constexpr (LIST) tile_of_seq(tiles_m, tiles_n, group_rows, seq0, tm, tn);
+  else tile_of_block(tiles_m, tiles_n, group_rows, tile_bid, tm, tn);
+  int m0 = tm * BM, n0 = tn * BN;
   unsigned my_xcc = 0;
   if constexpr (KSPLIT == 2) {
     if (p.splitk_local) {
@@ -476,10 +510,14 @@
       TFKB_WAIT_BARRIER(0);
       return;
     }
-  } else {
-    la.init(p.A, p.lda, A_KC ? p.M : p.K, m0, A_KC ? p.M : ((p.M + 7) & ~7), a_klim, tid);
-    lb.init(p.B, p.ldb, B_KC ? p.N : p.K, n0, B_KC ? p.N : ((p.N + 7) & ~7), b_klim, tid);
-  }
+  }
+  auto init_loaders = [&]() {
+    if constexpr (LOADERS == 0) {
+      la.init(p.A, p.lda, A_KC ? p.M : p.K, m0, A_KC ? p.M : ((p.M + 7) & ~7), a_klim, tid);
+      lb.init(p.B, p.ldb, B_KC ? p.N : p.K, n0, B_KC ? p.N : ((p.N + 7) & ~7), b_klim, tid);
+    }
+  };
+  init_loaders();
   typename std::conditional<NPL == 3, Frag3<A_KC, BM, FM>, Frag<A_KC, BM, FM, BKT>>::type qa;
   typename std::conditional<NPL == 3, Frag3<B_KC, BN, FN>, Frag<B_KC, BN, FN, BKT>>::type qb;
   qa.init(lane, wm * FM);
@@ -487,20 +525,22 @@
 
   f32x16 acc[FM][FN];
   f32x16 acc2[NPL == 3 ? FM : 1][NPL == 3 ? FN : 1];
-#pragma unroll
-  for (int a = 0; a < FM; ++a)
-#pragma unroll
-    for (int b = 0; b < FN; ++b)
-#pragma unroll
-      for (int r = 0; r < 16; ++r) acc[a][b][r] = 0.f;
-  if constexpr (NPL == 3) {
+  auto zero_acc = [&]() {
 #pragma unroll
     for (int a = 0; a < FM; ++a)
 #pragma unroll
       for (int b = 0; b < FN; ++b)
 #pragma unroll
-        for (int r = 0; r < 16; ++r) acc2[a][b][r] = 0.f;
-  }
+        for (int r = 0; r < 16; ++r) acc[a][b][r] = 0.f;
+    if constexpr (NPL == 3) {
+#pragma unroll
+      for (int a = 0; a < FM; ++a)
+#pragma unroll
+        for (int b = 0; b < FN; ++b)
+#pragma unroll
+          for (int r = 0; r < 16; ++r) acc2[a][b][r] = 0.f;
+    }
+  };
 
   auto piece_g = [&](auto guard, int j, int slot, int kt) {
     if (TFKB_ABL & 2) return;
@@ -519,14 +559,16 @@
     }
   };
   auto piece = [&](int j, int slot, int kt) { piece_g(std::true_type(), j, slot, kt); };
-#pragma unroll
-  for (int t = 0; t < NS - 1; ++t)
-#pragma unroll
-    for (int j = 0; j < NP; ++j) piece(j, t, t);
   constexpr int NPH = NPL == 3 ? NP / 2 : 0;
-#pragma unroll
-  for (int j = 0; j < NPH; ++j) piece(j, NS - 1, NS - 1);
-  TFKB_WAIT_BARRIER((NS - 2) * NP + NPH);
+  auto prologue = [&]() {
+#pragma unroll
+    for (int t = 0; t < NS - 1; ++t)
+#pragma unroll
+      for (int j = 0; j < NP; ++j) piece(j, t, t);
+#pragma unroll
+    for (int j = 0; j < NPH; ++j) piece(j, NS - 1, NS - 1);
+    TFKB_WAIT_BARRIER((NS - 2) * NP + NPH);
+  };
 
   bf16x8 fa[2][NPL][FM], fb[2][NPL][FN];
   auto read_frags = [&](int buf, const char* st, int ks) {
@@ -593,302 +635,347 @@
           acc[a][b] = __builtin_amdgcn_mfma_f32_32x32x16_bf16(fa[cur][0][a], fb[cur][0][b], acc[a][b], 0, 0, 0);
     }
   };
+  constexpr bool CHAIN = LIST && NPL == 3 && TFK_X3_M16 == 0 && SCHED == 0;
+  const int nlist = LIST ? ntiles : 1;
+  float* const red = reinterpret_cast<float*>(smem + (LIST ? NS * STAGE : 0));
+  bool primed = false;
   int rs = 0, ws = NS - 1;
-  if constexpr (SCHED == 2) {
-    static_assert(WAVES_M * WAVES_N == 8, "two waves per SIMD");
-    const int group = wave >> 2;
-    bf16x8 wa[KSPT][FM], wb[KSPT][FN];
-    if (group == 1) {
-      __builtin_amdgcn_sched_barrier(0);
-      asm volatile("s_barrier" : : : "memory");
-      __builtin_amdgcn_sched_barrier(0);
-    }
+#pragma unroll 1
+  for (int ti = 0; ti < nlist; ++ti) {
+    TFKB_TL(0, ti);
+    if (!primed) {
+      if (ti > 0) {
+        tile_of_seq(tiles_m, tiles_n, group_rows, seq0 + ti, tm, tn);
+        m0 = tm * BM;
+        n0 = tn * BN;
+        init_loaders();
+      }
+      prologue();
+      rs = 0;
+      ws = NS - 1;
+    }
+    zero_acc();
+    const bool chain_next = CHAIN && nk >= NS && ti + 1 < nlist;
+    const int tm_out = tm, m0_out = m0, n0_out = n0;
+    if constexpr (SCHED == 2) {
+      static_assert(WAVES_M * WAVES_N == 8, "two waves per SIMD");
+      const int group = wave >> 2;
+      bf16x8 wa[KSPT][FM], wb[KSPT][FN];
+      if (group == 1) {
+        __builtin_amdgcn_sched_barrier(0);
+        asm volatile("s_barrier" : : : "memory");
+        __builtin_amdgcn_sched_barrier(0);
+      }
+#pragma unroll 1
+      for (int kt = 0; kt < nk; ++kt) {
+        const char* st = smem + rs * STAGE;
+#pragma unroll
+        for (int ks = 0; ks < KSPT; ++ks) {
+#pragma unroll
+          for (int a = 0; a < FM; ++a) wa[ks][a] = qa.read(st, a, ks);
+#pragma unroll
+          for (int b = 0; b < FN; ++b) wb[ks][b] = qb.read(st + A_BYTES, b, ks);
+        }
+#pragma unroll
+        for (int j = 0; j < NP; ++j) piece(j, ws, kt + NS - 1);
+        __builtin_amdgcn_sched_barrier(0);
+        TFKB_WAIT_BARRIER((NS - 2) * NP);
+        __builtin_amdgcn_sched_barrier(0);
+#pragma unroll
+        for (int ks = 0; ks < KSPT; ++ks)
+#pragma unroll
+          for (int a = 0; a < FM; ++a)
+#pragma unroll
+            for (int b = 0; b < FN; ++b)
+              acc[a][b] = __builtin_amdgcn_mfma_f32_32x32x16_bf16(wa[ks][a], wb[ks][b], acc[a][b], 0, 0, 0);
+        rs = rs + 1 == NS ? 0 : rs + 1;
+        ws = ws + 1 == NS ? 0 : ws + 1;
+        __builtin_amdgcn_sched_barrier(0);
+        asm volatile("s_barrier" : : : "memory");
+        __builtin_amdgcn_sched_barrier(0);
+      }
+      if (group == 0) {
+        __builtin_amdgcn_sched_barrier(0);
+        asm volatile("s_barrier" : : : "memory");
+        __builtin_amdgcn_sched_barrier(0);
+      }
+    } else if constexpr (NPL == 3 && TFK_X3_M16 != 0) {
+      static_assert(KSPT == 2, "fp32-emulating contraction: 32 k per ring slot");
+      constexpr int FM16 = 2 * FM, FN16 = 2 * FN;
+      typedef float f32x4 __attribute__((ext_vector_type(4)));
+      Frag3M<A_KC, BM, FM16> ma;
+      Frag3M<B_KC, BN, FN16> mb;
+      ma.init(lane, wm * FM16);
+      mb.init(lane, wn * FN16);
+      f32x4 c1[FM16][FN16], c2[FM16][FN16];
+#pragma unroll
+      for (int a = 0; a < FM16; ++a)
+#pragma unroll
+        for (int b = 0; b < FN16; ++b) {
+          c1[a][b] = f32x4{0.f, 0.f, 0.f, 0.f};
+          c2[a][b] = f32x4{0.f, 0.f, 0.f, 0.f};
+        }
+      bf16x8 ga[3][FM16], gb[3][FN16], gb0n[FN16];
+      auto rd_a = [&](const decltype(ma)& r, int pl) {
+#pragma unroll
+        for (int a = 0; a < FM16; ++a) ga[pl][a] = r.read(smem, a, pl);
+      };
+      auto rd_b = [&](const decltype(mb)& r, int pl, bf16x8 (&dst)[FN16]) {
+#pragma unroll
+        for (int b = 0; b < FN16; ++b) dst[b] = r.read(smem, b, pl);
+      };
+      auto mm = [&](int pa, int pb) {
+#pragma unroll
+        for (int a = 0; a < FM16; ++a)
+#pragma unroll
+          for (int b = 0; b < FN16; ++b) {
+            if (pa + pb == 0) c1[a][b] = __builtin_amdgcn_mfma_f32_16x16x32_bf16(ga[0][a], gb[0][b], c1[a][b], 0, 0, 0);
+            else c2[a][b] = __builtin_amdgcn_mfma_f32_16x16x32_bf16(ga[pa][a], gb[pb][b], c2[a][b], 0, 0, 0);
+          }
+        __builtin_amdgcn_sched_barrier(0);
+      };
+      auto pieces = [&](auto guard, int part, int j0, int j1, int slot, int tile) {
+#pragma unroll
+        for (int j = j0 + part * (j1 - j0) / 3; j < j0 + (part + 1) * (j1 - j0) / 3; ++j) piece_g(guard, j, slot, tile);
+      };
+      {
+        const auto r0a = ma.at(0);
+        const auto r0b = mb.at(NPL * A_BYTES);
+        rd_a(r0a, 0);
+        rd_b(r0b, 0, gb[0]);
+        rd_b(r0b, 1, gb[1]);
+        rd_b(r0b, 2, gb[2]);
+      }
+      const int n_fast = max(0, min(nk, nk_full - NS));
+      auto iteration = [&](auto guard, int kt) {
+        const auto ra = ma.at(rs * STAGE);
+        rd_a(ra, 1);
+        pieces(guard, 0, NPH, NP, ws, kt + NS - 1);
+        mm(0, 0);
+        rd_a(ra, 2);
+        pieces(guard, 1, NPH, NP, ws, kt + NS - 1);
+        mm(0, 1);
+        pieces(guard, 2, NPH, NP, ws, kt + NS - 1);
+        mm(0, 2);
+        TFKB_WAIT_BARRIER((NS - 2) * NP);
+        rs = rs + 1 == NS ? 0 : rs + 1;
+        ws = ws + 1 == NS ? 0 : ws + 1;
+        const bool fetch = kt + 1 < nk;
+        const auto na = ma.at(rs * STAGE);
+        const auto nb = mb.at(rs * STAGE + NPL * A_BYTES);
+        if (fetch) {
+          rd_a(na, 0);
+          rd_b(nb, 0, gb0n);
+        }
+        pieces(guard, 0, 0, NPH, ws, kt + NS);
+        mm(1, 0);
+        if (fetch) rd_b(nb, 2, gb[2]);
+        pieces(guard, 1, 0, NPH, ws, kt + NS);
+        mm(1, 1);
+        if (fetch) rd_b(nb, 1, gb[1]);
+        pieces(guard, 2, 0, NPH, ws, kt + NS);
+        mm(2, 0);
+        if (fetch) {
+#pragma unroll
+          for (int b = 0; b < FN16; ++b) gb[0][b] = gb0n[b];
+        }
+      };
+#pragma unroll 1
+      for (int kt = 0; kt < n_fast; ++kt) iteration(std::false_type(), kt);
+#pragma unroll 1
+      for (int kt = n_fast; kt < nk; ++kt) iteration(std::true_type(), kt);
+      {
+        const int src = (16 * h + (i & 15)) * 4;
+#pragma unroll
+        for (int a = 0; a < FM; ++a)
+#pragma unroll
+          for (int b = 0; b < FN; ++b)
+#pragma unroll
+            for (int r = 0; r < 16; ++r) {
+              const int addr = src + (((r >> 2) & 1) ? 128 : 0);
+              const f32x4& t0 = c1[2 * a + (r >> 3)][2 * b], &u0 = c2[2 * a + (r >> 3)][2 * b];
+              const f32x4& t1 = c1[2 * a + (r >> 3)][2 * b + 1], &u1 = c2[2 * a + (r >> 3)][2 * b + 1];
+              const float v0 = __builtin_bit_cast(float, __builtin_amdgcn_ds_bpermute(addr, __builtin_bit_cast(int, t0[r & 3] + u0[r & 3])));
+              const float v1 = __builtin_bit_cast(float, __builtin_amdgcn_ds_bpermute(addr, __builtin_bit_cast(int, t1[r & 3] + u1[r & 3])));
+              acc[a][b][r] = (i & 16) ? v1 : v0;
+            }
+      }
+    } else if constexpr (NPL == 3) {
+      static_assert(KSPT == 2, "fp32-emulating contraction: 32 k per ring slot");
+      constexpr int PA[6] = {2, 1, 0, 1, 0, 0}, PB[6] = {0, 1, 2, 0, 1, 0};
+      auto step3 = [&](auto guard, int cur, bool fetch, const decltype(qa)& ra, const decltype(qb)& rb, int nks, int j0, int j1,
+                       int slot, int tile) {
+#pragma unroll
+        for (int c = 0; c < 6; ++c) {
+          if (c < 3 && fetch && !(TFKB_ABL & 4)) {
+#pragma unroll
+            for (int a = 0; a < FM; ++a) fa[cur ^ 1][PA[c]][a] = ra.read(smem, a, nks, PA[c]);
+#pragma unroll
+            for (int b = 0; b < FN; ++b) fb[cur ^ 1][PB[c]][b] = rb.read(smem, b, nks, PB[c]);
+          }
+#pragma unroll
+          for (int j = j0 + c * (j1 - j0) / 6; j < j0 + (c + 1) * (j1 - j0) / 6; ++j) piece_g(guard, j, slot, tile);
+          if (TFKB_ABL & 1) {
+#pragma unroll
+            for (int a = 0; a < FM; ++a) asm volatile("" : : "v"(fa[cur][PA[c]][a]));
+#pragma unroll
+            for (int b = 0; b < FN; ++b) asm volatile("" : : "v"(fb[cur][PB[c]][b]));
+          } else {
+#pragma unroll
+            for (int a = 0; a < FM; ++a)
+#pragma unroll
+              for (int b = 0; b < FN; ++b) {
+                if (c < 5)
+                  acc2[a][b] = __builtin_amdgcn_mfma_f32_32x32x16_bf16(fa[cur][PA[c]][a], fb[cur][PB[c]][b], acc2[a][b], 0, 0, 0);
+                else
+                  acc[a][b] = __builtin_amdgcn_mfma_f32_32x32x16_bf16(fa[cur][PA[c]][a], fb[cur][PB[c]][b], acc[a][b], 0, 0, 0);
+              }
+          }
+          __builtin_amdgcn_sched_barrier(0);
+        }
+      };
+      if (!primed) read_frags(0, smem, 0);
+      const int n_fast = max(0, min(nk, nk_full - NS));
+      auto iteration = [&](auto guard, int t1, int t2, bool fetch, bool switch_tile) {
+        const auto ra = qa.at(rs * STAGE);
+        const auto rb = qb.at(rs * STAGE + NPL * A_BYTES);
+        step3(guard, 0, true, ra, rb, 1, NPH, NP, ws, t1);
+        TFKB_WAIT_BARRIER((NS - 2) * NP);
+        rs = rs + 1 == NS ? 0 : rs + 1;
+        ws = ws + 1 == NS ? 0 : ws + 1;
+        if constexpr (CHAIN) {
+          if (switch_tile) {
+            tile_of_seq(tiles_m, tiles_n, group_rows, seq0 + ti + 1, tm, tn);
+            m0 = tm * BM;
+            n0 = tn * BN;
+            init_loaders();
+          }
+        }
+        const auto na = qa.at(rs * STAGE);
+        const auto nb = qb.at(rs * STAGE + NPL * A_BYTES);
+        step3(guard, 1, fetch, na, nb, 0, 0, NPH, ws, t2);
+      };
+      const int n_own = chain_next ? nk - NS : nk;
+      TFKB_TL(1, ti);
+#pragma unroll 1
+      for (int kt = 0; kt < n_fast; ++kt) iteration(std::false_type(), kt + NS - 1, kt + NS, kt + 1 < nk, false);
+#pragma unroll 1
+      for (int kt = n_fast; kt < n_own; ++kt) iteration(std::true_type(), kt + NS - 1, kt + NS, kt + 1 < nk, false);
+      if constexpr (CHAIN) {
+        if (chain_next) {
+          iteration(std::true_type(), nk - 1, 0, true, true);
+#pragma unroll 1
+          for (int t = 0; t < NS - 1; ++t) iteration(std::true_type(), t, t + 1, true, false);
+        }
+      }
+      TFKB_TL(2, ti);
+    } else {
+    read_frags(0, smem, 0);
 #pragma unroll 1
     for (int kt = 0; kt < nk; ++kt) {
       const char* st = smem + rs * STAGE;
 #pragma unroll
-      for (int ks = 0; ks < KSPT; ++ks) {
-#pragma unroll
-        for (int a = 0; a < FM; ++a) wa[ks][a] = qa.read(st, a, ks);
-#pragma unroll
-        for (int b = 0; b < FN; ++b) wb[ks][b] = qb.read(st + A_BYTES, b, ks);
-      }
-#pragma unroll
-      for (int j = 0; j < NP; ++j) piece(j, ws, kt + NS - 1);
-      __builtin_amdgcn_sched_barrier(0);
-      TFKB_WAIT_BARRIER((NS - 2) * NP);
-      __builtin_amdgcn_sched_barrier(0);
-#pragma unroll
-      for (int ks = 0; ks < KSPT; ++ks)
-#pragma unroll
-        for (int a = 0; a < FM; ++a)
-#pragma unroll
-          for (int b = 0; b < FN; ++b)
-            acc[a][b] = __builtin_amdgcn_mfma_f32_32x32x16_bf16(wa[ks][a], wb[ks][b], acc[a][b], 0, 0, 0);
-      rs = rs + 1 == NS ? 0 : rs + 1;
-      ws = ws + 1 == NS ? 0 : ws + 1;
-      __builtin_amdgcn_sched_barrier(0);
-      asm volatile("s_barrier" : : : "memory");
-      __builtin_amdgcn_sched_barrier(0);
-    }
-    if (group == 0) {
-      __builtin_amdgcn_sched_barrier(0);
-      asm volatile("s_barrier" : : : "memory");
-      __builtin_amdgcn_sched_barrier(0);
-    }
-  } else if constexpr (NPL == 3 && TFK_X3_M16 != 0) {
-    static_assert(KSPT == 2, "fp32-emulating contraction: 32 k per ring slot");
-    constexpr int FM16 = 2 * FM, FN16 = 2 * FN;
-    typedef float f32x4 __attribute__((ext_vector_type(4)));
-    Frag3M<A_KC, BM, FM16> ma;
-    Frag3M<B_KC, BN, FN16> mb;
-    ma.init(lane, wm * FM16);
-    mb.init(lane, wn * FN16);
-    f32x4 c1[FM16][FN16], c2[FM16][FN16];
-#pragma unroll
-    for (int a = 0; a < FM16; ++a)
-#pragma unroll
-      for (int b = 0; b < FN16; ++b) {
-        c1[a][b] = f32x4{0.f, 0.f, 0.f, 0.f};
-        c2[a][b] = f32x4{0.f, 0.f, 0.f, 0.f};
-      }
-    bf16x8 ga[3][FM16], gb[3][FN16], gb0n[FN16];
-    auto rd_a = [&](const decltype(ma)& r, int pl) {
-#pragma unroll
-      for (int a = 0; a < FM16; ++a) ga[pl][a] = r.read(smem, a, pl);
-    };
-    auto rd_b = [&](const decltype(mb)& r, int pl, bf16x8 (&dst)[FN16]) {
-#pragma unroll
-      for (int b = 0; b < FN16; ++b) dst[b] = r.read(smem, b, pl);
-    };
-    auto mm = [&](int pa, int pb) {
-#pragma unroll
-      for (int a = 0; a < FM16; ++a)
-#pragma unroll
-        for (int b = 0; b < FN16; ++b) {
-          if (pa + pb == 0) c1[a][b] = __builtin_amdgcn_mfma_f32_16x16x32_bf16(ga[0][a], gb[0][b], c1[a][b], 0, 0, 0);
-          else c2[a][b] = __builtin_amdgcn_mfma_f32_16x16x32_bf16(ga[pa][a], gb[pb][b], c2[a][b], 0, 0, 0);
-        }
-      __builtin_amdgcn_sched_barrier(0);
-    };
-    auto pieces = [&](auto guard, int part, int j0, int j1, int slot, int tile) {
-#pragma unroll
-      for (int j = j0 + part * (j1 - j0) / 3; j < j0 + (part + 1) * (j1 - j0) / 3; ++j) piece_g(guard, j, slot, tile);
-    };
-    {
-      const auto r0a = ma.at(0);
-      const auto r0b = mb.at(NPL * A_BYTES);
-      rd_a(r0a, 0);
-      rd_b(r0b, 0, gb[0]);
-      rd_b(r0b, 1, gb[1]);
-      rd_b(r0b, 2, gb[2]);
-    }
-    const int n_fast = max(0, min(nk, nk_full - NS));
-    auto iteration = [&](auto guard, int kt) {
-      const auto ra = ma.at(rs * STAGE);
-      rd_a(ra, 1);
-      pieces(guard, 0, NPH, NP, ws, kt + NS - 1);
-      mm(0, 0);
-      rd_a(ra, 2);
-      pieces(guard, 1, NPH, NP, ws, kt + NS - 1);
-      mm(0, 1);
-      pieces(guard, 2, NPH, NP, ws, kt + NS - 1);
-      mm(0, 2);
+      for (int ks = 0; ks < KSPT - 1; ++ks) {
+        const int cur = ks & 1;
+        read_frags(cur ^ 1, st, ks + 1);
+#pragma unroll
+        for (int j = ks * NP / (KSPT - 1); j < (ks + 1) * NP / (KSPT - 1); ++j) piece(j, ws, kt + NS - 1);
+        mfma_step(cur);
+        __builtin_amdgcn_sched_barrier(0);
+      }
       TFKB_WAIT_BARRIER((NS - 2) * NP);
       rs = rs + 1 == NS ? 0 : rs + 1;
       ws = ws + 1 == NS ? 0 : ws + 1;
-      const bool fetch = kt + 1 < nk;
-      const auto na = ma.at(rs * STAGE);
-      const auto nb = mb.at(rs * STAGE + NPL * A_BYTES);
-      if (fetch) {
-        rd_a(na, 0);
-        rd_b(nb, 0, gb0n);
-      }
-      pieces(guard, 0, 0, NPH, ws, kt + NS);
-      mm(1, 0);
-      if (fetch) rd_b(nb, 2, gb[2]);
-      pieces(guard, 1, 0, NPH, ws, kt + NS);
-      mm(1, 1);
-      if (fetch) rd_b(nb, 1, gb[1]);
-      pieces(guard, 2, 0, NPH, ws, kt + NS);
-      mm(2, 0);
-      if (fetch) {
-#pragma unroll
-        for (int b = 0; b < FN16; ++b) gb[0][b] = gb0n[b];
-      }
-    };
-#pragma unroll 1
-    for (int kt = 0; kt < n_fast; ++kt) iteration(std::false_type(), kt);
-#pragma unroll 1
-    for (int kt = n_fast; kt < nk; ++kt) iteration(std::true_type(), kt);
-    {
-      const int src = (16 * h + (i & 15)) * 4;
+      if (kt + 1 < nk) read_frags(0, smem + rs * STAGE, 0);
+      mfma_step((KSPT - 1) & 1);
+      __builtin_amdgcn_sched_barrier(0);
+    }
+    }
+    if (!chain_next) TFKB_WAIT_BARRIER(0);
+    if constexpr (NPL == 3) {
 #pragma unroll
       for (int a = 0; a < FM; ++a)
 #pragma unroll
         for (int b = 0; b < FN; ++b)
 #pragma unroll
-          for (int r = 0; r < 16; ++r) {
-            const int addr = src + (((r >> 2) & 1) ? 128 : 0);
-            const f32x4& t0 = c1[2 * a + (r >> 3)][2 * b], &u0 = c2[2 * a + (r >> 3)][2 * b];
-            const f32x4& t1 = c1[2 * a + (r >> 3)][2 * b + 1], &u1 = c2[2 * a + (r >> 3)][2 * b + 1];
-            const float v0 = __builtin_bit_cast(float, __builtin_amdgcn_ds_bpermute(addr, __builtin_bit_cast(int, t0[r & 3] + u0[r & 3])));
-            const float v1 = __builtin_bit_cast(float, __builtin_amdgcn_ds_bpermute(addr, __builtin_bit_cast(int, t1[r & 3] + u1[r & 3])));
-            acc[a][b][r] = (i & 16) ? v1 : v0;
+          for (int r = 0; r < 16; ++r) acc[a][b][r] += acc2[a][b][r];
+    }
+    if constexpr (KSPLIT == 2) {
+      typedef float f32x4 __attribute__((ext_vector_type(4)));
+      unsigned* flags = reinterpret_cast<unsigned*>(p.splitk_ws);
+      const int tile = tm * tiles_n + tn;
+      constexpr int kSys = 1 | (1 << 4);
+      __amdgpu_buffer_rsrc_t part = __builtin_amdgcn_make_buffer_rsrc(
+          (void*)(p.splitk_ws + kSplitFlagWords + (size_t)tile * (BM * BN)), 0, BM * BN * 4, 0x00020000);
+      unsigned* sh = reinterpret_cast<unsigned*>(smem);
+      if (tid == 0) {
+        sh[0] = __hip_atomic_fetch_add(&flags[2 * tile], 1u, __ATOMIC_RELAXED, __HIP_MEMORY_SCOPE_AGENT);
+        sh[1] = p.splitk_local ? __hip_atomic_load(&flags[kSplitXccWord + 2 * tile + (khalf ^ 1)], __ATOMIC_RELAXED, __HIP_MEMORY_SCOPE_AGENT)
+                               : 0u;
+      }
+      __syncthreads();
+      const bool first = sh[0] == 0;
+      if (first) {
+        const bool same_xcd = p.splitk_local && sh[1] == my_xcc + 1;
+        if (same_xcd) {
+#pragma unroll
+          for (int a = 0; a < FM; ++a)
+#pragma unroll
+            for (int b = 0; b < FN; ++b)
+#pragma unroll
+              for (int q = 0; q < 4; ++q)
+                __builtin_amdgcn_raw_buffer_store_b128(
+                    __builtin_bit_cast(u32x4, f32x4{acc[a][b][4 * q], acc[a][b][4 * q + 1], acc[a][b][4 * q + 2], acc[a][b][4 * q + 3]}),
+                    part, ((((wave * FM + a) * FN + b) * 4 + q) * 64 + lane) * 16, 0, 0);
+        } else {
+#pragma unroll
+          for (int a = 0; a < FM; ++a)
+#pragma unroll
+            for (int b = 0; b < FN; ++b)
+#pragma unroll
+              for (int q = 0; q < 4; ++q)
+                __builtin_amdgcn_raw_buffer_store_b128(
+                    __builtin_bit_cast(u32x4, f32x4{acc[a][b][4 * q], acc[a][b][4 * q + 1], acc[a][b][4 * q + 2], acc[a][b][4 * q + 3]}),
+                    part, ((((wave * FM + a) * FN + b) * 4 + q) * 64 + lane) * 16, 0, kSys);
+        }
+        asm volatile("s_waitcnt vmcnt(0)" : : : "memory");
+        __syncthreads();
+        if (tid == 0) __hip_atomic_store(&flags[2 * tile + 1], 1u, __ATOMIC_RELAXED, __HIP_MEMORY_SCOPE_AGENT);
+        return;
+      }
+      if (tid == 0) {
+        int spin = 0;
+        for (; spin < (1 << 23) && __hip_atomic_load(&flags[2 * tile + 1], __ATOMIC_RELAXED, __HIP_MEMORY_SCOPE_AGENT) == 0; ++spin)
+          __builtin_amdgcn_s_sleep(2);
+        if (spin == (1 << 23) && p.err) __hip_atomic_store(p.err, 1u, __ATOMIC_RELAXED, __HIP_MEMORY_SCOPE_SYSTEM);
+        __hip_atomic_store(&flags[2 * tile], 0u, __ATOMIC_RELAXED, __HIP_MEMORY_SCOPE_AGENT);
+        __hip_atomic_store(&flags[2 * tile + 1], 0u, __ATOMIC_RELAXED, __HIP_MEMORY_SCOPE_AGENT);
+        __hip_atomic_store(&flags[kSplitXccWord + 2 * tile], 0u, __ATOMIC_RELAXED, __HIP_MEMORY_SCOPE_AGENT);
+        __hip_atomic_store(&flags[kSplitXccWord + 2 * tile + 1], 0u, __ATOMIC_RELAXED, __HIP_MEMORY_SCOPE_AGENT);
+      }
+      __syncthreads();
+#pragma unroll
+      for (int a = 0; a < FM; ++a)
+#pragma unroll
+        for (int b = 0; b < FN; ++b)
+#pragma unroll
+          for (int q = 0; q < 4; ++q) {
+            const f32x4 o = __builtin_bit_cast(
+                f32x4, __builtin_amdgcn_raw_buffer_load_b128(part, ((((wave * FM + a) * FN + b) * 4 + q) * 64 + lane) * 16, 0, kSys));
+            acc[a][b][4 * q] += o.x;
+            acc[a][b][4 * q + 1] += o.y;
+            acc[a][b][4 * q + 2] += o.z;
+            acc[a][b][4 * q + 3] += o.w;
           }
-    }
-  } else if constexpr (NPL == 3) {
-    static_assert(KSPT == 2, "fp32-emulating contraction: 32 k per ring slot");
-    constexpr int PA[6] = {2, 1, 0, 1, 0, 0}, PB[6] = {0, 1, 2, 0, 1, 0};
-    auto step3 = [&](auto guard, int cur, bool fetch, const decltype(qa)& ra, const decltype(qb)& rb, int nks, int j0, int j1,
-                     int slot, int tile) {
-#pragma unroll
-      for (int c = 0; c < 6; ++c) {
-        if (c < 3 && fetch && !(TFKB_ABL & 4)) {
-#pragma unroll
-          for (int a = 0; a < FM; ++a) fa[cur ^ 1][PA[c]][a] = ra.read(smem, a, nks, PA[c]);
-#pragma unroll
-          for (int b = 0; b < FN; ++b) fb[cur ^ 1][PB[c]][b] = rb.read(smem, b, nks, PB[c]);
-        }
-#pragma unroll
-        for (int j = j0 + c * (j1 - j0) / 6; j < j0 + (c + 1) * (j1 - j0) / 6; ++j) piece_g(guard, j, slot, tile);
-        if (TFKB_ABL & 1) {
-#pragma unroll
-          for (int a = 0; a < FM; ++a) asm volatile("" : : "v"(fa[cur][PA[c]][a]));
-#pragma unroll
-          for (int b = 0; b < FN; ++b) asm volatile("" : : "v"(fb[cur][PB[c]][b]));
-        } else {
-#pragma unroll
-          for (int a = 0; a < FM; ++a)
-#pragma unroll
-            for (int b = 0; b < FN; ++b) {
-              if (c < 5)
-                acc2[a][b] = __builtin_amdgcn_mfma_f32_32x32x16_bf16(fa[cur][PA[c]][a], fb[cur][PB[c]][b], acc2[a][b], 0, 0, 0);
-              else
-                acc[a][b] = __builtin_amdgcn_mfma_f32_32x32x16_bf16(fa[cur][PA[c]][a], fb[cur][PB[c]][b], acc[a][b], 0, 0, 0);
-            }
-        }
-        __builtin_amdgcn_sched_barrier(0);
-      }
-    };
-    read_frags(0, smem, 0);
-    const int n_fast = max(0, min(nk, nk_full - NS));
-    auto iteration = [&](auto guard, int kt) {
-      const auto ra = qa.at(rs * STAGE);
-      const auto rb = qb.at(rs * STAGE + NPL * A_BYTES);
-      step3(guard, 0, true, ra, rb, 1, NPH, NP, ws, kt + NS - 1);
-      TFKB_WAIT_BARRIER((NS - 2) * NP);
-      rs = rs + 1 == NS ? 0 : rs + 1;
-      ws = ws + 1 == NS ? 0 : ws + 1;
-      const auto na = qa.at(rs * STAGE);
-      const auto nb = qb.at(rs * STAGE + NPL * A_BYTES);
-      step3(guard, 1, kt + 1 < nk, na, nb, 0, 0, NPH, ws, kt + NS);
-    };
-#pragma unroll 1
-    for (int kt = 0; kt < n_fast; ++kt) iteration(std::false_type(), kt);
-#pragma unroll 1
-    for (int kt = n_fast; kt < nk; ++kt) iteration(std::true_type(), kt);
-  } else {
-  read_frags(0, smem, 0);
-#pragma unroll 1
-  for (int kt = 0; kt < nk; ++kt) {
-    const char* st = smem + rs * STAGE;
-#pragma unroll
-    for (int ks = 0; ks < KSPT - 1; ++ks) {
-      const int cur = ks & 1;
-      read_frags(cur ^ 1, st, ks + 1);
-#pragma unroll
-      for (int j = ks * NP / (KSPT - 1); j < (ks + 1) * NP / (KSPT - 1); ++j) piece(j, ws, kt + NS - 1);
-      mfma_step(cur);
-      __builtin_amdgcn_sched_barrier(0);
-    }
-    TFKB_WAIT_BARRIER((NS - 2) * NP);
-    rs = rs + 1 == NS ? 0 : rs + 1;
-    ws = ws + 1 == NS ? 0 : ws + 1;
-    if (kt + 1 < nk) read_frags(0, smem + rs * STAGE, 0);
-    mfma_step((KSPT - 1) & 1);
-    __builtin_amdgcn_sched_barrier(0);
-  }
-  }
-  TFKB_WAIT_BARRIER(0);
-  if constexpr (NPL == 3) {
-#pragma unroll
-    for (int a = 0; a < FM; ++a)
-#pragma unroll
-      for (int b = 0; b < FN; ++b)
-#pragma unroll
-        for (int r = 0; r < 16; ++r) acc[a][b][r] += acc2[a][b][r];
-  }
-  if constexpr (KSPLIT == 2) {
-    typedef float f32x4 __attribute__((ext_vector_type(4)));
-    unsigned* flags = reinterpret_cast<unsigned*>(p.splitk_ws);
-    const int tile = tm * tiles_n + tn;
-    constexpr int kSys = 1 | (1 << 4);
-    __amdgpu_buffer_rsrc_t part = __builtin_amdgcn_make_buffer_rsrc(
-        (void*)(p.splitk_ws + kSplitFlagWords + (size_t)tile * (BM * BN)), 0, BM * BN * 4, 0x00020000);
-    unsigned* sh = reinterpret_cast<unsigned*>(smem);
-    if (tid == 0) {
-      sh[0] = __hip_atomic_fetch_add(&flags[2 * tile], 1u, __ATOMIC_RELAXED, __HIP_MEMORY_SCOPE_AGENT);
-      sh[1] = p.splitk_local ? __hip_atomic_load(&flags[kSplitXccWord + 2 * tile + (khalf ^ 1)], __ATOMIC_RELAXED, __HIP_MEMORY_SCOPE_AGENT)
-                             : 0u;
-    }
-    __syncthreads();
-    const bool first = sh[0] == 0;
-    if (first) {
-      const bool same_xcd = p.splitk_local && sh[1] == my_xcc + 1;
-      if (same_xcd) {
-#pragma unroll
-        for (int a = 0; a < FM; ++a)
-#pragma unroll
-          for (int b = 0; b < FN; ++b)
-#pragma unroll
-            for (int q = 0; q < 4; ++q)
-              __builtin_amdgcn_raw_buffer_store_b128(
-                  __builtin_bit_cast(u32x4, f32x4{acc[a][b][4 * q], acc[a][b][4 * q + 1], acc[a][b][4 * q + 2], acc[a][b][4 * q + 3]}),
-                  part, ((((wave * FM + a) * FN + b) * 4 + q) * 64 + lane) * 16, 0, 0);
-      } else {
-#pragma unroll
-        for (int a = 0; a < FM; ++a)
-#pragma unroll
-          for (int b = 0; b < FN; ++b)
-#pragma unroll
-            for (int q = 0; q < 4; ++q)
-              __builtin_amdgcn_raw_buffer_store_b128(
-                  __builtin_bit_cast(u32x4, f32x4{acc[a][b][4 * q], acc[a][b][4 * q + 1], acc[a][b][4 * q + 2], acc[a][b][4 * q + 3]}),
-                  part, ((((wave * FM + a) * FN + b) * 4 + q) * 64 + lane) * 16, 0, kSys);
-      }
-      asm volatile("s_waitcnt vmcnt(0)" : : : "memory");
       __syncthreads();
-      if (tid == 0) __hip_atomic_store(&flags[2 * tile + 1], 1u, __ATOMIC_RELAXED, __HIP_MEMORY_SCOPE_AGENT);
-      return;
-    }
-    if (tid == 0) {
-      int spin = 0;
-      for (; spin < (1 << 23) && __hip_atomic_load(&flags[2 * tile + 1], __ATOMIC_RELAXED, __HIP_MEMORY_SCOPE_AGENT) == 0; ++spin)
-        __builtin_amdgcn_s_sleep(2);
-      if (spin == (1 << 23) && p.err) __hip_atomic_store(p.err, 1u, __ATOMIC_RELAXED, __HIP_MEMORY_SCOPE_SYSTEM);
-      __hip_atomic_store(&flags[2 * tile], 0u, __ATOMIC_RELAXED, __HIP_MEMORY_SCOPE_AGENT);
-      __hip_atomic_store(&flags[2 * tile + 1], 0u, __ATOMIC_RELAXED, __HIP_MEMORY_SCOPE_AGENT);
-      __hip_atomic_store(&flags[kSplitXccWord + 2 * tile], 0u, __ATOMIC_RELAXED, __HIP_MEMORY_SCOPE_AGENT);
-      __hip_atomic_store(&flags[kSplitXccWord + 2 * tile + 1], 0u, __ATOMIC_RELAXED, __HIP_MEMORY_SCOPE_AGENT);
-    }
-    __syncthreads();
-#pragma unroll
-    for (int a = 0; a < FM; ++a)
-#pragma unroll
-      for (int b = 0; b < FN; ++b)
-#pragma unroll
-        for (int q = 0; q < 4; ++q) {
-          const f32x4 o = __builtin_bit_cast(
-              f32x4, __builtin_amdgcn_raw_buffer_load_b128(part, ((((wave * FM + a) * FN + b) * 4 + q) * 64 + lane) * 16, 0, kSys));
-          acc[a][b][4 * q] += o.x;
-          acc[a][b][4 * q + 1] += o.y;
-          acc[a][b][4 * q + 2] += o.z;
-          acc[a][b][4 * q + 3] += o.w;
-        }
-    __syncthreads();
-  }
-  epilogue<EPI, WAVES_M, WAVES_N, FM, FN>(p, acc, tiles_m, tm, m0, n0, wm, wn, i, h, reinterpret_cast<float*>(smem));
+    }
+    epilogue<EPI, WAVES_M, WAVES_N, FM, FN, CBUF>(p, acc, tiles_m, tm_out, m0_out, n0_out, wm, wn, i, h, red);
+    TFKB_TL(3, ti);
+    if constexpr (LIST) {
+      primed = chain_next;
+      if (!chain_next && ti + 1 < nlist) __syncthreads();
+    }
+  }
 }
 
 template <bool A_KC, bool B_KC, int EPI, int WAVES_M, int WAVES_N, int FM, int FN, int NS, int BKT = 64, int SCHED = 0,
@@ -1091,17 +1178,29 @@
 template <int EPI_NT, int EPI_TN, int WN>
 __global__ void __launch_bounds__(WN == 2 ? 256 : 512)
 gemm_bf16x3_dual_kernel(GemmArgsB p1, GemmArgsB p2, int tiles_m1, int tiles_n1, int group1, int tiles_m2, int tiles_n2, int group2,
-                        int tn_first) {
+                        int tn_first, int per) {
   extern __shared__ __attribute__((aligned(16))) char smem[];
   const int n1 = tiles_m1 * tiles_n1, n2 = tiles_m2 * tiles_n2;
   const int b = blockIdx.x;
-  const bool nt = tn_first ? b >= n2 : b < n1;
-  if (nt)
-    dma_tile<true, true, EPI_NT, 2, WN ? WN : 2, 2, WN ? 4 / WN : 2, 3, 32, 0, 3, 1, WN ? 0 : 4>(p1, tiles_m1, tiles_n1, group1,
-                                                                                              tn_first ? b - n2 : b, smem);
+  constexpr bool LIST = WN != 0;
+  constexpr int WNN = WN ? WN : 2, FNN = WN ? 4 / WN : 2, LD = WN ? 0 : 4;
+  const int n_long = tn_first ? n2 : n1;
+  if (b < n_long) {
+    if (tn_first) dma_tile<false, false, EPI_TN, 2, WNN, 2, FNN, 3, 32, 0, 3, 1, LD, false, true>(p2, tiles_m2, tiles_n2, group2, b, smem);
+    else dma_tile<true, true, EPI_NT, 2, WNN, 2, FNN, 3, 32, 0, 3, 1, LD, false, true>(p1, tiles_m1, tiles_n1, group1, b, smem);
+    return;
+  }
+  int seq0 = 0, count = 1;
+  if constexpr (LIST) {
+    x3::dual_block_tiles(tn_first ? n1 : n2, per, b - n_long, seq0, count);
+    if (count == 0) return;
+  }
+  if (tn_first)
+    dma_tile<true, true, EPI_NT, 2, WNN, 2, FNN, 3, 32, 0, 3, 1, LD, LIST, true>(p1, tiles_m1, tiles_n1, group1, b - n_long, smem, seq0,
+                                                                                 count);
   else
-    dma_tile<false, false, EPI_TN, 2, WN ? WN : 2, 2, WN ? 4 / WN : 2, 3, 32, 0, 3, 1, WN ? 0 : 4>(p2, tiles_m2, tiles_n2, group2,
-                                                                                                tn_first ? b : b - n1, smem);
+    dma_tile<false, false, EPI_TN, 2, WNN, 2, FNN, 3, 32, 0, 3, 1, LD, LIST, true>(p2, tiles_m2, tiles_n2, group2, b - n_long, smem, seq0,
+                                                                                  count);
 }
 
 struct CfgB {
@@ -1347,7 +1446,7 @@
 namespace {
 template <int EPI_NT, int EPI_TN, int WN>
 int launch_x3_dual(const GemmArgsB& a, const GemmArgsB& w, hipStream_t stream) {
-  constexpr size_t lds = (size_t)3 * 3 * (128 + 128) * 32 * 2;
+  constexpr size_t lds = (size_t)3 * 3 * (128 + 128) * 32 * 2 + 2 * 2 * 128 * sizeof(float);
   auto kern = &gemm_bf16x3_dual_kernel<EPI_NT, EPI_TN, WN>;
   static bool attr_done = false;
   if (!attr_done) {
@@ -1356,8 +1455,13 @@
     attr_done = true;
   }
   const int tma = (a.M + 127) / 128, tna = (a.N + 127) / 128, tmw = (w.M + 127) / 128, tnw = (w.N + 127) / 128;
-  hipLaunchKernelGGL(kern, dim3(tma * tna + tmw * tnw), dim3(WN == 2 ? 256 : 512), lds, stream, a, w, tma, tna, pick_group_rows(tma, tna, 128, 128),
-                     tmw, tnw, pick_group_rows(tmw, tnw, 128, 128), w.K > a.K ? 1 : 0);
+  const int tn_first = w.K > a.K ? 1 : 0;
+  const int n_long = tn_first ? tmw * tnw : tma * tna, n_short = tn_first ? tma * tna : tmw * tnw;
+  const int nk_long = ((tn_first ? w.K : a.K) + 31) / 32, nk_short = ((tn_first ? a.K : w.K) + 31) / 32;
+  const int per = WN == 0 ? 1 : x3::dual_tiles_per_block(n_long, nk_long, n_short, nk_short);
+  const int blocks = n_long + (WN == 0 ? n_short : x3::dual_short_blocks(n_short, per));
+  hipLaunchKernelGGL(kern, dim3(blocks), dim3(WN == 2 ? 256 : 512), lds, stream, a, w, tma, tna, pick_group_rows(tma, tna, 128, 128), tmw, tnw,
+                     pick_group_rows(tmw, tnw, 128, 128), tn_first, per);
   return (int)hipGetLastError();
 }
 bool x3_operands_ok(const GemmArgsB& p, long a_rows, long b_rows) {
@@ -1372,6 +1476,7 @@
   static const bool on = !getenv("TFK_BF16X3_DUAL") || atoi(getenv("TFK_BF16X3_DUAL")) != 0;
   const long tiles = (long)((nt.M + 127) / 128) * ((nt.N + 127) / 128) + (long)((tn.M + 127) / 128) * ((tn.N + 127) / 128);
   if (!on || tiles < 256) return -1;
+  if ((long)nt.M * nt.ldc * 4 >= (1L << 31) || (long)tn.M * tn.ldc * 4 >= (1L << 31)) return -1;
   const int key = (nt.epi == EPI_DACT ? 2 : 0) + (tn.epi == EPI_ACCUM ? 1 : 0);
   switch (key) {
 #define TFK_X3_DUAL(E1, E2)                                                                \
diff --git a/tfkaldi_amd/csrc/x3_layout.h b/tfkaldi_amd/csrc/x3_layout.h
--- a/tfkaldi_amd/csrc/x3_layout.h
+++ b/tfkaldi_amd/csrc/x3_layout.h
@@ -92,6 +92,30 @@
   return 128 * (X & ~1) + hi * 2 * (EXT / 32 * 384);
 }
 
+constexpr int kXcds = 8;
+constexpr int kCus = 256;
+X3_HD int dual_tiles_per_block(int n_long, int nk_long, int n_short, int nk_short) {
+  int per = (nk_long + (nk_short - 1) / 2) / nk_short;
+  if (per < 1) per = 1;
+  while (per > 1 && n_long + (n_short + per - 1) / per < kCus) --per;
+  return per;
+}
+X3_HD void dual_block_tiles(int n_short, int per, int g, int& seq0, int& count) {
+  const int xcd = g % kXcds, j = g / kXcds;
+  const int q = n_short / kXcds, r = n_short % kXcds;
+  const int start = xcd < r ? xcd * (q + 1) : r * (q + 1) + (xcd - r) * q;
+  const int cnt = q + (xcd < r ? 1 : 0);
+  const int left = cnt - j * per;
+  seq0 = start + j * per;
+  count = left <= 0 ? 0 : left < per ? left : per;
+}
+X3_HD int dual_short_blocks(int n_short, int per) {
+  const int q = n_short / kXcds, r = n_short % kXcds;
+  if (q == 0) return r;
+  const int j_q = (q + per - 1) / per, j_q1 = (q + 1 + per - 1) / per;
+  return (r > 0 && j_q1 > j_q) ? kXcds * j_q + r : kXcds * j_q;
+}
+
 #if defined(__HIPCC__)
 __device__ __forceinline__ void split3(float x, uint16_t& p1, uint16_t& p2, uint16_t& p3) {
   const uint32_t ux = __builtin_bit_cast(uint32_t, x);
```

New measurement: 929,400, median of 6. 1.1% higher.
